# ushasigh/srsran-edgeric-5g

Measured on AMD Instinct MI355X. Metric: pdsch_slots_per_sec, higher is better.
Workload: dtype u32 bit-packed GF(2) + bf16 grid + f32 IQ

## Files before the change

### srsran-edgeric-5g_amd/csrc/ldpc_device.h

```cpp
#pragma once

#include "bits_device.h"

namespace nrphy {

constexpr int LDPC_MAX_WPB   = 12;
constexpr int LDPC_LIN_WORDS = (68 * 384) / 32 + 2;
constexpr int LDPC_DBL_WORDS = 2 * 22 * LDPC_MAX_WPB;

template <bool ALIGNED>
__device__ __forceinline__ uint32_t rot_word(const uint32_t* a, uint32_t base, uint32_t zc, uint32_t s, uint32_t j)
{
  uint32_t start = s + 32u * j;
  start          = start >= zc ? start - zc : start;
  if (ALIGNED) {
    const uint32_t wpb = zc >> 5, bw = base >> 5;
    const uint32_t w0 = start >> 5, sh = s & 31u;
    const uint32_t w1 = (w0 + 1u == wpb) ? 0u : w0 + 1u;
    return (a[bw + w0] << sh) | ((a[bw + w1] >> 1) >> (31u - sh));
  }
  uint32_t n_valid = zc - 32u * j;
  n_valid          = n_valid > 32u ? 32u : n_valid;
  uint32_t first   = zc - start;
  first            = first > n_valid ? n_valid : first;
  uint32_t v       = ext32(a, base + start) & topmask(first);
  if (first < n_valid) {
    v |= (ext32(a, base) & topmask(n_valid - first)) >> first;
  }
  return v;
}

struct LdpcScratch {
  uint32_t aux[4][LDPC_MAX_WPB + 1];
  uint32_t sum[LDPC_MAX_WPB + 2];
  uint32_t p0[LDPC_MAX_WPB + 2];
};

template <bool ALIGNED>
__device__ __forceinline__ void put_block_word(uint32_t* lin, uint32_t node, uint32_t zc, uint32_t j, uint32_t v)
{
  uint32_t pos = node * zc + 32u * j;
  if (ALIGNED) {
    lin[pos >> 5] = v;
  } else {
    uint32_t n_valid = zc - 32u * j;
    or_bits_lds(lin, pos, v, n_valid > 32u ? 32u : n_valid);
  }
}

constexpr uint32_t LDPC_GRAPH_ROWPTR = 48;

__device__ __forceinline__ void stage_graph(const LiftedGraph* g, uint32_t nof_rows, uint32_t* gbuf, uint32_t lane)
{
  if (lane <= nof_rows) {
    gbuf[lane] = g->row_ptr[lane];
  }
  const uint32_t nedges = g->row_ptr[nof_rows];
  for (uint32_t e = lane; e < nedges; e += WAVE) {
    gbuf[LDPC_GRAPH_ROWPTR + e] = g->edge[e];
  }
}

struct GraphRows {
  static constexpr uint32_t TRIPS = (MAX_BG_EDGES + WAVE - 1) / WAVE;
  uint32_t row_ptr, nedges, edge[TRIPS];
  __device__ __forceinline__ void fetch(const LiftedGraph* g, uint32_t nof_rows, uint32_t lane)
  {
    row_ptr = lane <= nof_rows ? g->row_ptr[lane] : 0u;
    nedges  = g->row_ptr[nof_rows];
#pragma unroll
    for (uint32_t k = 0; k != TRIPS; ++k) {
      edge[k] = lane + WAVE * k < nedges ? g->edge[lane + WAVE * k] : 0u;
    }
  }
  __device__ __forceinline__ void store(uint32_t nof_rows, uint32_t* gbuf, uint32_t lane) const
  {
    if (lane <= nof_rows) {
      gbuf[lane] = row_ptr;
    }
#pragma unroll
    for (uint32_t k = 0; k != TRIPS; ++k) {
      if (lane + WAVE * k < nedges) {
        gbuf[LDPC_GRAPH_ROWPTR + lane + WAVE * k] = edge[k];
      }
    }
  }
};

template <bool ALIGNED>
__device__ __forceinline__ uint32_t row_word(const uint32_t* gbuf, const uint32_t* lin, uint32_t zc, uint32_t m,
                                             uint32_t j)
{
  uint32_t acc = 0;
  for (uint32_t e = gbuf[m], end = gbuf[m + 1]; e != end; ++e) {
    uint32_t edge = gbuf[LDPC_GRAPH_ROWPTR + e];
    acc ^= rot_word<ALIGNED>(lin, edge >> 16, zc, edge & 0xFFFFu, j);
  }
  return acc;
}

__device__ __forceinline__ uint32_t core_row_word_dbl(const uint32_t* gbuf, const uint32_t* dbl, uint32_t m, uint32_t j)
{
  uint32_t       acc = 0;
  const uint8_t* at  = reinterpret_cast<const uint8_t*>(dbl) + 4u * j;
  uint32_t       e = gbuf[m], end = gbuf[m + 1];
  for (; e + 4u <= end; e += 4u) {
    uint32_t        edge[4];
    u32x2_unaligned w[4];
#pragma unroll
    for (int k = 0; k != 4; ++k) {
      edge[k] = gbuf[LDPC_GRAPH_ROWPTR + e + k];
    }
#pragma unroll
    for (int k = 0; k != 4; ++k) {
      w[k] = *reinterpret_cast<const u32x2_unaligned*>(at + (edge[k] >> 16));
    }
#pragma unroll
    for (int k = 0; k != 4; ++k) {
      acc ^= __builtin_amdgcn_alignbit(w[k].x, w[k].y, edge[k]);
    }
  }
  for (; e != end; ++e) {
    const uint32_t        edge = gbuf[LDPC_GRAPH_ROWPTR + e];
    const u32x2_unaligned w    = *reinterpret_cast<const u32x2_unaligned*>(at + (edge >> 16));
    acc ^= __builtin_amdgcn_alignbit(w.x, w.y, edge);
  }
  return acc;
}

__device__ __forceinline__ void ldpc_double_blocks(const uint32_t* lin, uint32_t kb, uint32_t wpb, uint32_t* dbl, uint32_t lane)
{
  const uint32_t magic = (65536u + wpb - 1u) / wpb;
  for (uint32_t item = lane; item < kb * wpb; item += WAVE) {
    const uint32_t n = __umul24(item, magic) >> 16;
    const uint32_t v = lin[item];
    dbl[item + __umul24(n, wpb)]       = v;
    dbl[item + __umul24(n, wpb) + wpb] = v;
  }
}

template <bool ALIGNED>
__device__ inline void ldpc_encode_wave_impl(const LiftedGraph* g, const uint32_t* gbuf, uint32_t kb, uint32_t zc,
                                             uint32_t nof_rows, uint32_t* lin, uint32_t* dbl, LdpcScratch* sc, uint32_t lane)
{
  const uint32_t wpb = (zc + 31u) >> 5;
  if (ALIGNED) {
    ldpc_double_blocks(lin, kb, wpb, dbl, lane);
    wave_sync();
  }
  const uint32_t wpb_magic = (65536u + wpb - 1u) / wpb;
  for (uint32_t item = lane; item < 4u * wpb; item += WAVE) {
    const uint32_t m = __umul24(item, wpb_magic) >> 16, j = item - __umul24(m, wpb);
    sc->aux[m][j] = ALIGNED ? core_row_word_dbl(gbuf, dbl, m, j) : row_word<ALIGNED>(gbuf, lin, zc, m, j);
  }
  wave_sync();
  if (lane < wpb) {
    sc->sum[lane] = sc->aux[0][lane] ^ sc->aux[1][lane] ^ sc->aux[2][lane] ^ sc->aux[3][lane];
  }
  if (lane == 0) {
    sc->sum[wpb] = 0;
    sc->p0[wpb]  = 0;
  }
  wave_sync();
  uint32_t p0w = 0;
  if (lane < wpb) {
    uint32_t b = g->core_b;
    p0w        = rot_word<ALIGNED>(sc->sum, 0, zc, b == 0 ? 0 : zc - b, lane);
    sc->p0[lane] = p0w;
  }
  wave_sync();
  if (lane < wpb) {
    uint32_t p1 = sc->aux[0][lane] ^ rot_word<ALIGNED>(sc->p0, 0, zc, g->core_s0, lane);
    uint32_t p3 = sc->aux[3][lane] ^ rot_word<ALIGNED>(sc->p0, 0, zc, g->core_s3, lane);
    uint32_t p2 = (g->core_mid == 1) ? (sc->aux[2][lane] ^ p3) : (sc->aux[1][lane] ^ p1);
    put_block_word<ALIGNED>(lin, kb + 0, zc, lane, p0w);
    put_block_word<ALIGNED>(lin, kb + 1, zc, lane, p1);
    put_block_word<ALIGNED>(lin, kb + 2, zc, lane, p2);
    put_block_word<ALIGNED>(lin, kb + 3, zc, lane, p3);
  }
  wave_sync();
  uint32_t ext_items = (nof_rows > 4u ? nof_rows - 4u : 0u) * wpb;
  for (uint32_t item = lane; item < ext_items; item += WAVE) {
    uint32_t m = item / wpb, j = item - m * wpb;
    m += 4u;
    put_block_word<ALIGNED>(lin, kb + m, zc, j, row_word<ALIGNED>(gbuf, lin, zc, m, j));
  }
  wave_sync();
}

__device__ inline void ldpc_encode_wave(const LiftedGraph* g, const uint32_t* gbuf, uint32_t kb, uint32_t zc,
                                        uint32_t nof_rows, uint32_t* lin, uint32_t* dbl, LdpcScratch* sc, uint32_t lane)
{
  if ((zc & 31u) == 0) {
    ldpc_encode_wave_impl<true>(g, gbuf, kb, zc, nof_rows, lin, dbl, sc, lane);
  } else {
    ldpc_encode_wave_impl<false>(g, gbuf, kb, zc, nof_rows, lin, dbl, sc, lane);
  }
}

}
```

### srsran-edgeric-5g_amd/csrc/nrphy_host.cpp

```cpp
#include "nrphy_host_internal.h"
#include "nrphy_trace.h"

#include <algorithm>
#include <cmath>
#include <complex>
#include <cstdlib>
#include <cstring>
#include <array>
#include <map>
#include <mutex>
#include <new>
#include <unordered_map>
#include <vector>

using namespace nrphy;

namespace {

struct nr_ldpc_edge_t {
  uint8_t  row;
  uint8_t  col;
  uint16_t shift[8];
};
#include "nr_ldpc_bg.inc"
// ... 682 lines not shown
}

extern "C" int nrphy_destroy(nrphy_ctx_t* ctx)
{
  if (ctx == nullptr) {
    return NRPHY_OK;
  }
  (void)hipSetDevice(ctx->device);
  (void)hipFree(ctx->d_graphs);
  (void)hipFree(ctx->d_gold);
  (void)hipFree(ctx->d_tbcrc);
  for (void* b : ctx->scratch) {
    (void)hipFree(b);
  }
  for (DecoderGraph* g : ctx->d_dec_graph) {
    (void)hipFree(g);
  }
  for (uint32_t* a : ctx->d_dec_addr) {
    (void)hipFree(a);
  }
  for (auto& kv : ctx->d_dec_crc) {
    (void)hipFree(kv.second);
  }
  for (auto& kv : ctx->d_tb_crc_w) {
    (void)hipFree(kv.second);
  }
  (void)hipFree(ctx->d_x1);
  (void)hipFree(ctx->d_prach);
  for (auto& kv : ctx->d_twiddle) {
    (void)hipFree(kv.second);
  }
  if (ctx->stream) {
    (void)hipStreamDestroy(ctx->stream);
  }
  delete ctx;
  return NRPHY_OK;
}

extern "C" int nrphy_synchronize(nrphy_ctx_t* ctx, void* stream)
{
  if (ctx == nullptr) {
    return NRPHY_ERR_ARGUMENT;
  }
  HIP_TRY(hipStreamSynchronize(stream ? (hipStream_t)stream : ctx->stream));
  return NRPHY_OK;
}

const float2* get_twiddle(nrphy_ctx* ctx, uint32_t size)
{
  if (!dft_size_supported(size)) {
    return nullptr;
  }
  std::lock_guard<std::recursive_mutex> lock(ctx->host_mutex);
  auto it = ctx->d_twiddle.find(size);
  if (it != ctx->d_twiddle.end()) {
    return it->second;
  }
  std::vector<float2> tw(size);
  for (uint32_t k = 0; k != size; ++k) {
    double ang = 2.0 * M_PI * (double)k / (double)size;
    tw[k]      = make_float2((float)std::cos(ang), (float)std::sin(ang));
  }
  float2* d = nullptr;
  if (upload(&d, tw.data(), tw.size() * sizeof(float2)) != hipSuccess) {
    return nullptr;
  }
  ctx->d_twiddle[size] = d;
  return d;
}

namespace {

void append_allocation_signature(const nrphy_pdsch_pdu_t& pdu, std::vector<uint64_t>& sig)
{
  sig.insert(sig.end(), std::begin(pdu.prb_mask), std::end(pdu.prb_mask));
  sig.push_back(((uint64_t)pdu.start_symbol_index << 48) | ((uint64_t)pdu.nof_symbols << 40) |
                ((uint64_t)pdu.nof_cdm_groups_without_data << 36) | ((uint64_t)pdu.nof_layers << 32) |
                pdu.dmrs_symbol_mask);
  sig.push_back(((uint64_t)pdu.bwp_start_rb << 32) | ((uint64_t)pdu.bwp_size_rb << 8) | pdu.nof_reserved);
  for (unsigned r = 0; r != pdu.nof_reserved; ++r) {
    sig.insert(sig.end(), std::begin(pdu.reserved[r].prb_mask), std::end(pdu.reserved[r].prb_mask));
    sig.push_back(((uint64_t)pdu.reserved[r].re_mask << 32) | pdu.reserved[r].symbol_mask);
  }
}

struct ReMapping {
  uint32_t sym_re_start[NRPHY_NSYMB + 1];
  uint32_t sym_kind[NRPHY_NSYMB];
  uint32_t sym_arg[NRPHY_NSYMB];
};

}

struct PlanShapeCache {
  struct Remap {
    ReMapping             m;
    std::vector<uint16_t> table;
  };
  struct Zero {
    std::vector<ZeroSeg> segs;
    uint32_t             nof_long = 0;
  };
  std::map<std::vector<uint64_t>, Remap> remap;
  std::map<std::vector<uint64_t>, Zero>  zero;
  static constexpr size_t MAX_ENTRIES = 256;
};

PlanShapeCache* plan_shape_cache_create()
{
  return new (std::nothrow) PlanShapeCache;
}
void plan_shape_cache_destroy(PlanShapeCache* c)
{
  delete c;
}

namespace {

struct EncodeOnly {
  uint32_t nof_re;
  uint32_t nref;
};

int plan_create(nrphy_ctx_t* ctx, uint32_t n_pdu, const nrphy_pdsch_pdu_t* pdus, const uint64_t* tb_offset,
                const uint32_t* grid_index, uint32_t nof_grids, uint32_t grid_nof_ports, uint32_t grid_nof_subc,
                const EncodeOnly* enc, nrphy_pdsch_plan_t** out, PlanPlacement* place = nullptr);

}

int nrphy_pdsch_plan_create_placed(nrphy_ctx_t* ctx, uint32_t n_pdu, const nrphy_pdsch_pdu_t* pdus, const uint64_t* tb_offset,
                                   const uint32_t* grid_index, uint32_t nof_grids, uint32_t grid_nof_ports,
                                   uint32_t grid_nof_subc, PlanPlacement* place, nrphy_pdsch_plan_t** out)
{
  return plan_create(ctx, n_pdu, pdus, tb_offset, grid_index, nof_grids, grid_nof_ports, grid_nof_subc, nullptr, out, place);
}

extern "C" int nrphy_pdsch_plan_create(nrphy_ctx_t* ctx, uint32_t n_pdu, const nrphy_pdsch_pdu_t* pdus,
                                       const uint64_t* tb_offset, const uint32_t* grid_index, uint32_t nof_grids,
                                       uint32_t grid_nof_ports, uint32_t grid_nof_subc, nrphy_pdsch_plan_t** out)
{
  return plan_create(ctx, n_pdu, pdus, tb_offset, grid_index, nof_grids, grid_nof_ports, grid_nof_subc, nullptr, out);
}

namespace {

int plan_create(nrphy_ctx_t* ctx, uint32_t n_pdu, const nrphy_pdsch_pdu_t* pdus, const uint64_t* tb_offset,
                const uint32_t* grid_index, uint32_t nof_grids, uint32_t grid_nof_ports, uint32_t grid_nof_subc,
                const EncodeOnly* enc, nrphy_pdsch_plan_t** out, PlanPlacement* place)
{
  if (ctx == nullptr || out == nullptr || (n_pdu != 0 && (pdus == nullptr || tb_offset == nullptr)) ||
      grid_nof_ports == 0 || grid_nof_ports > NRPHY_MAX_PORTS || grid_nof_subc == 0 || grid_nof_subc % 12 != 0 ||
      grid_nof_subc > NRPHY_MAX_RB * 12) {
    return NRPHY_ERR_ARGUMENT;
  }
  *out = nullptr;
  if (place == nullptr) {
    HIP_TRY(hipSetDevice(ctx->device));
  }
  nrphy_pdsch_plan* plan = new (std::nothrow) nrphy_pdsch_plan;
  if (plan == nullptr) {
    return NRPHY_ERR_CAPACITY;
  }
  PlanShapeCache* shapes = place ? place->cache : nullptr;
  if (shapes != nullptr && shapes->remap.size() + shapes->zero.size() > PlanShapeCache::MAX_ENTRIES) {
    shapes->remap.clear();
    shapes->zero.clear();
  }
  plan->ctx            = ctx;
  plan->nof_grids      = nof_grids;
  plan->grid_nof_ports = grid_nof_ports;
  plan->grid_nof_subc  = grid_nof_subc;
  plan->encode_only    = enc != nullptr;

  std::vector<CbWork>   work;
  std::vector<DmrsWork> dmrs;
  std::vector<CrcWork>  crc_work;
  std::vector<uint64_t> remap_sig;
  std::map<std::vector<uint64_t>, ReMapping> remap_cache;
  std::vector<ScrWork>  scr_work;
  std::unordered_map<SeqKey, SeqShare, SeqKeyHash> seq_shares;
  std::vector<uint8_t>  seq_fresh;
  uint32_t              seed_slots = 0;
  uint64_t              seq_words = 0;
  uint64_t              seq_words_sum = 0;
  bool                  seq_words_fit = true;
  std::vector<std::vector<uint32_t>> pdus_of_grid(nof_grids);
  std::vector<float>    weights;
  std::vector<uint16_t> re_table;
  std::vector<uint8_t>  mask(grid_nof_subc);
  std::vector<uint16_t> list;
  uint64_t              cw_bits = 0;
  int                   status  = NRPHY_OK;

  for (uint32_t i = 0; i != n_pdu && status == NRPHY_OK; ++i) {
    const nrphy_pdsch_pdu_t& pdu = pdus[i];
    if (enc == nullptr ? nrphy_pdsch_validate(&pdu) != NRPHY_OK
                       : (pdu.qm < 2 || pdu.qm > 8 || (pdu.qm & 1U) || pdu.rv > 3 || pdu.nof_layers == 0 ||
                          pdu.nof_layers > NRPHY_MAX_LAYERS || pdu.tb_size_bytes == 0 ||
                          pdu.tb_size_bytes > NRPHY_MAX_TB_BYTES || (pdu.ldpc_base_graph != 1 && pdu.ldpc_base_graph != 2))) {
      status = NRPHY_ERR_INVALID_PDU;
      break;
    }
    const uint32_t g = grid_index ? grid_index[i] : 0;
    if (g >= nof_grids || pdu.nof_ports > grid_nof_ports || (tb_offset[i] & 3U) != 0 ||
        (enc == nullptr && 12U * (unsigned)(mask_highest(pdu.prb_mask) + 1) > grid_nof_subc)) {
      status = NRPHY_ERR_ARGUMENT;
      break;
    }
    PduDev pd;
    std::memset(&pd, 0, sizeof(pd));
    unsigned nof_re = 0;
    remap_sig.clear();
    append_allocation_signature(pdu, remap_sig);
    auto cached = remap_cache.find(remap_sig);
    if (enc != nullptr) {
      nof_re = enc[i].nof_re;
      for (unsigned l = 0; l <= NRPHY_NSYMB; ++l) {
        pd.sym_re_start[l] = (l == NRPHY_NSYMB) ? nof_re : 0;
      }
    } else if (cached != remap_cache.end()) {
      std::memcpy(pd.sym_re_start, cached->second.sym_re_start, sizeof(pd.sym_re_start));
      std::memcpy(pd.sym_kind, cached->second.sym_kind, sizeof(pd.sym_kind));
      std::memcpy(pd.sym_arg, cached->second.sym_arg, sizeof(pd.sym_arg));
      nof_re = pd.sym_re_start[NRPHY_NSYMB];
    } else {
      PlanShapeCache::Remap        built;
      const PlanShapeCache::Remap* rel = nullptr;
      if (shapes != nullptr) {
        auto known = shapes->remap.find(remap_sig);
        if (known != shapes->remap.end()) {
          rel = &known->second;
        }
      }
      if (rel == nullptr) {
        for (unsigned l = 0; l != NRPHY_NSYMB; ++l) {
          built.m.sym_re_start[l] = nof_re;
          built.m.sym_arg[l]      = 0;
          data_re_mask(pdu, l, mask);
          list.clear();
          for (unsigned k = 0; k != grid_nof_subc; ++k) {
            if (mask[k]) {
              list.push_back((uint16_t)k);
            }
          }
          if (list.empty()) {
            built.m.sym_kind[l] = SYM_NONE;
          } else if ((unsigned)(list.back() - list.front()) + 1 == list.size()) {
            built.m.sym_kind[l] = SYM_CONTIGUOUS;
            built.m.sym_arg[l]  = list.front();
          } else {
            built.m.sym_kind[l] = SYM_TABLE;
            built.m.sym_arg[l]  = (uint32_t)built.table.size();
            for (unsigned lp = 0; lp != l; ++lp) {
              if (built.m.sym_kind[lp] == SYM_TABLE && built.m.sym_re_start[lp + 1] - built.m.sym_re_start[lp] == list.size() &&
                  std::equal(list.begin(), list.end(), built.table.begin() + built.m.sym_arg[lp])) {
                built.m.sym_arg[l] = built.m.sym_arg[lp];
                break;
              }
            }
            if (built.m.sym_arg[l] == built.table.size()) {
              built.table.insert(built.table.end(), list.begin(), list.end());
            }
          }
          nof_re += (unsigned)list.size();
          built.m.sym_re_start[l + 1] = nof_re;
        }
        rel = &built;
        if (shapes != nullptr) {
          rel = &shapes->remap.insert({remap_sig, built}).first->second;
        }
      }
      const uint32_t base = (uint32_t)re_table.size();
      re_table.insert(re_table.end(), rel->table.begin(), rel->table.end());
      std::memcpy(pd.sym_re_start, rel->m.sym_re_start, sizeof(pd.sym_re_start));
      std::memcpy(pd.sym_kind, rel->m.sym_kind, sizeof(pd.sym_kind));
      for (unsigned l = 0; l != NRPHY_NSYMB; ++l) {
        pd.sym_arg[l] = rel->m.sym_arg[l] + (rel->m.sym_kind[l] == SYM_TABLE ? base : 0U);
      }
      nof_re = pd.sym_re_start[NRPHY_NSYMB];
      ReMapping m;
      std::memcpy(m.sym_re_start, pd.sym_re_start, sizeof(m.sym_re_start));
      std::memcpy(m.sym_kind, pd.sym_kind, sizeof(m.sym_kind));
      std::memcpy(m.sym_arg, pd.sym_arg, sizeof(m.sym_arg));
      remap_cache.insert({remap_sig, m});
    }
    if (nof_re == 0) {
      status = NRPHY_ERR_INVALID_PDU;
      break;
    }
    nrphy_pdsch_derived_t d;
    derive(pdu, nof_re, d, enc ? &enc[i].nref : nullptr);
    if (d.lifting_size == 0 || d.nof_codeblocks > NRPHY_MAX_CODEBLOCKS || d.nof_codeblocks > nof_re ||
        d.rm_length_short == 0) {
      status = NRPHY_ERR_INVALID_PDU;
      break;
    }
    const unsigned kb = (pdu.ldpc_base_graph == 1) ? 22 : 10;
    pd.tb_offset      = tb_offset[i];
    pd.cw_bit_offset  = cw_bits;
    pd.tb_bytes       = pdu.tb_size_bytes;
    pd.grid_index     = g;
    pd.graph          = (pdu.ldpc_base_graph - 1) * NOF_LIFTING_SIZES + (uint32_t)lifting_position(d.lifting_size);
    pd.zc             = d.lifting_size;
    pd.kb             = kb;
    pd.K              = d.segment_length;
    pd.info_bits      = d.cb_info_bits;
    pd.filler         = d.nof_filler_bits;
    pd.tb_crc_bits    = d.nof_tb_crc_bits;
    pd.cb_crc_bits    = d.nof_cb_crc_bits;
    pd.zero_pad       = d.zero_pad;
    pd.C              = d.nof_codeblocks;
    pd.n_short        = d.nof_short_segments;
    pd.e_short        = d.rm_length_short;
    pd.e_long         = d.rm_length_long;
    pd.n_cb           = d.n_cb;
    pd.k0             = d.k0;
    pd.qm             = pdu.qm;
    pd.nof_layers     = pdu.nof_layers;
    pd.nof_ports      = pdu.nof_ports;
    pd.c_init         = (pdu.rnti << 15) + pdu.n_id;
    pd.nof_re         = nof_re;
    {
      const unsigned nsys = (kb - 2) * d.lifting_size;
      unsigned       fs = std::min(nsys - d.nof_filler_bits, d.n_cb), fe = std::min(nsys, d.n_cb);
      const unsigned flen = fe - fs, n_valid = d.n_cb - flen;
      const unsigned rank0 = d.k0 < fs ? d.k0 : (d.k0 < fe ? fs : d.k0 - flen);
      unsigned       last;
      if (rank0 + d.rm_length_long > n_valid) {
        last = d.n_cb - 1;
      } else {
        unsigned u = rank0 + d.rm_length_long - 1;
        last       = u < fs ? u : u + flen;
      }
      const unsigned nodes = divide_ceil(last + 1 + 2 * d.lifting_size, d.lifting_size);
      pd.nof_rows          = std::max(4U, nodes > kb ? nodes - kb : 0U);
    }
    {
      const float avg     = (pdu.qm == 2) ? 2.0F : (pdu.qm == 4) ? 10.0F : (pdu.qm == 6) ? 42.0F : 170.0F;
      float       scaling = std::sqrt(1 / avg);
      const float cfg     = std::pow(10.0F, -pdu.ratio_pdsch_data_to_sss_dB / 20.0F);
      if (std::isnormal(cfg)) {
        scaling *= cfg;
      }
      const unsigned nw      = 2 * pdu.nof_prg * pdu.nof_ports * pdu.nof_layers;
      pd.weights_offset      = (uint32_t)weights.size();
      for (unsigned k = 0; k != nw; ++k) {
        weights.push_back(pdu.precoding ? pdu.precoding[k] * scaling : 0.0F);
      }
      pd.dmrs_weights_offset = (uint32_t)weights.size();
      for (unsigned k = 0; k != nw; ++k) {
        weights.push_back(pdu.precoding ? pdu.precoding[k] : 0.0F);
      }
      pd.nof_prg       = pdu.nof_prg;
      pd.prg_size_subc = pdu.prg_size_rb * 12;
    }
    pd.dmrs_symbol_mask = pdu.dmrs_symbol_mask;
    pd.dmrs_zero_other_group = (pdu.nof_cdm_groups_without_data == 2 && (pdu.nof_layers + 1) / 2 == 1) ? 1U : 0U;
    pd.dmrs_ref_rb      = (pdu.ref_point == 1) ? pdu.bwp_start_rb : 0;
    {
      const float amp   = std::pow(10.0F, -pdu.ratio_pdsch_dmrs_to_sss_dB / 20.0F);
      pd.dmrs_amplitude = (float)(M_SQRT1_2 * (double)amp);
    }
    for (unsigned l = 0; l != NRPHY_NSYMB; ++l) {
      const uint64_t a  = (uint64_t)(14 * pdu.slot_index + l + 1) * (2 * pdu.scrambling_id + 1);
      pd.dmrs_c_init[l] = (uint32_t)(((a << 17) + (2 * pdu.scrambling_id + (pdu.n_scid ? 1 : 0))) & 0x7FFFFFFFULL);
      if ((pdu.dmrs_symbol_mask >> l) & 1U) {
        const uint32_t first = (uint32_t)mask_lowest(pdu.prb_mask), end = (uint32_t)mask_highest(pdu.prb_mask) + 1;
        for (uint32_t b = first; b < end; b += DMRS_PRB_CHUNK) {
          dmrs.push_back({i, l, b, std::min<uint32_t>(end, b + DMRS_PRB_CHUNK)});
        }
      }
    }
    for (unsigned w = 0; w != NRPHY_PRB_WORDS; ++w) {
      pd.prb_mask[2 * w]     = (uint32_t)pdu.prb_mask[w];
      pd.prb_mask[2 * w + 1] = (uint32_t)(pdu.prb_mask[w] >> 32);
    }
    pd.first_prb = (uint32_t)mask_lowest(pdu.prb_mask);
    pd.end_prb   = (uint32_t)mask_highest(pdu.prb_mask) + 1;
    if (pdu.nof_cdm_groups_without_data < (pdu.nof_layers + 1) / 2) {
      plan->dmrs_separate = true;
    }
    pdus_of_grid[g].push_back(i);
    const unsigned lq = pdu.nof_layers * pdu.qm;
    const size_t   work_before = work.size();
    for (unsigned cb = 0; cb != d.nof_codeblocks; ++cb) {
      const unsigned nre = ((cb < d.nof_short_segments) ? d.rm_length_short : d.rm_length_long) / lq;
      for (unsigned begin = 0; begin < nre; begin += RE_CHUNK) {
        const unsigned count = std::min<unsigned>(RE_CHUNK, nre - begin);
        work.push_back({i, cb, begin, count});
        {
          const uint64_t bit0 = (uint64_t)(cb < d.nof_short_segments ? cb * d.rm_length_short
                                                                     : d.nof_short_segments * d.rm_length_short +
                                                                           (cb - d.nof_short_segments) * d.rm_length_long) +
                                (uint64_t)begin * lq;
          const uint32_t need = std::max<uint32_t>(31U, (uint32_t)(((bit0 & 31U) + (uint64_t)count * lq + 31U) / 32U) + 1U);
          plan->lds_lin_words = std::max<uint32_t>(plan->lds_lin_words, (need + 3U) & ~3U);
        }
        plan->lds_symb_words = std::max<uint32_t>(plan->lds_symb_words,
                                                  (((count * pdu.nof_layers + 31) / 32) * 8 + 8 + 3) & ~3U);
      }
    }
    plan->lds_lin_words = std::max<uint32_t>(plan->lds_lin_words,
                                             ((((kb + pd.nof_rows) * d.lifting_size + 31) / 32) + 2 + 3) & ~3U);
    plan->lds_graph_words = std::max<uint32_t>(
        plan->lds_graph_words, (48U + ctx->graphs[pd.graph].row_ptr[std::min<uint32_t>(pd.nof_rows, MAX_BG_ROWS)] + 3U) & ~3U);
    pd.scr_words  = (d.codeword_bits + 31U) / 32U + 1U + 31U;
    pd.dmrs_seq_words  = (12U * (pd.end_prb - pd.dmrs_ref_rb) + 31U) / 32U + 1U;
    {
      const uint32_t nof_dmrs_words = (uint32_t)(((uint64_t)pd.dmrs_seq_words * (unsigned)__builtin_popcount(pdu.dmrs_symbol_mask) + 3U) & ~3ULL);
      const uint32_t nof_items      = (uint32_t)(work.size() - work_before);
      uint8_t        fresh          = (uint8_t)(SEQ_NEW_SCR | (nof_dmrs_words != 0 ? SEQ_NEW_DMRS : 0));
      SeqShare       share          = {seed_slots, (uint32_t)seq_words, (uint32_t)plan->scr_words};
      if (n_pdu != 1) {
        SeqKey key;
        key.scr  = {pd.c_init, pd.C, pd.n_short, pd.e_short, pd.e_long, lq};
        key.dmrs = {};
        key.dmrs[0] = pdu.dmrs_symbol_mask;
        key.dmrs[1] = pd.dmrs_seq_words;
        for (unsigned l = 0; l != NRPHY_NSYMB; ++l) {
          key.dmrs[2 + l] = ((pdu.dmrs_symbol_mask >> l) & 1U) ? pd.dmrs_c_init[l] : 0U;
        }
        auto both = seq_shares.find(key);
        if (both != seq_shares.end()) {
          share = both->second;
          fresh = 0;
        } else {
          SeqKey half = key;
          half.dmrs   = {};
          half.dmrs[1] = ~0U;
          auto scr_known = seq_shares.insert({half, share});
          if (!scr_known.second) {
            share.seed_first      = scr_known.first->second.seed_first;
            share.scr_word_offset = scr_known.first->second.scr_word_offset;
            fresh &= (uint8_t)~SEQ_NEW_SCR;
          }
          if (nof_dmrs_words != 0) {
            half     = key;
            half.scr = {};
            auto dmrs_known = seq_shares.insert({half, share});
            if (!dmrs_known.second) {
              share.dmrs_seq_offset = dmrs_known.first->second.dmrs_seq_offset;
              fresh &= (uint8_t)~SEQ_NEW_DMRS;
            }
          }
          seq_shares.insert({key, share});
        }
      }
      pd.seed_first      = share.seed_first;
      pd.scr_word_offset = share.scr_word_offset;
      pd.dmrs_seq_offset = share.dmrs_seq_offset;
      if (fresh & SEQ_NEW_SCR) {
        seed_slots += nof_items;
        seq_words_sum += pd.scr_words;
        seq_words += (pd.scr_words + 15U) & ~15ULL;
        seq_words_fit = seq_words_fit && pd.scr_words <= (uint32_t)GOLD_X1_WORDS && seq_words <= 0xFFFFFFFFULL;
        ++plan->n_scr_seq;
      }
      if (fresh & SEQ_NEW_DMRS) {
        plan->scr_words += nof_dmrs_words;
        ++plan->n_dmrs_seq;
      }
      seq_fresh.push_back(fresh);
    }
    plan->n_cb += d.nof_codeblocks;
    plan->cw_offset.push_back(cw_bits);
    cw_bits += (d.codeword_bits + 31U) & ~31ULL;
    plan->pdus.push_back(pd);
  }
  if (status == NRPHY_OK) {
    const uint32_t parts_big = ctx->tune.scr_parts_big > 0 ? (uint32_t)std::min((int)SCR_PARTS, ctx->tune.scr_parts_big) : 1U;
    const uint32_t parts_max = plan->n_scr_seq >= 128 ? parts_big : SCR_PARTS;
    for (uint32_t i = 0; i != n_pdu; ++i) {
      const PduDev&  pd       = plan->pdus[i];
      const uint32_t own_dmrs = (seq_fresh[i] & SEQ_NEW_DMRS) ? 1U : 0U;
      if (seq_fresh[i] & SEQ_NEW_SCR) {
        const uint32_t parts = std::min<uint32_t>(parts_max, std::max<uint32_t>(1, pd.scr_words >> 11));
        const uint32_t chunk = divide_ceil(pd.scr_words, parts);
        for (uint32_t first = 0, k = 0; first < pd.scr_words; first += chunk, ++k) {
          scr_work.push_back({i, first, std::min(chunk, pd.scr_words - first), k == 0 ? own_dmrs : 0U});
        }
      } else if (own_dmrs) {
        scr_work.push_back({i, 0U, 0U, 1U});
      }
    }
  }
  for (uint32_t i = 0; i != n_pdu && status == NRPHY_OK; ++i) {
    PduDev&         pd = plan->pdus[i];
    const CrcField& f  = (pd.tb_crc_bits == 16) ? CRC16_FIELD : CRC24A_FIELD;
    const uint32_t  n  = pd.tb_bytes;
    const uint32_t  regions = divide_ceil(n, TB_CRC_REGION_BYTES);
    const uint32_t  want  = std::max<uint32_t>(1, std::min<uint32_t>(regions, TB_CRC_TARGET_WORK / std::max<uint32_t>(1, n_pdu)));
    uint32_t        per   = std::min<uint32_t>(TB_CRC_MAX_REGIONS_PER_WORK, divide_ceil(regions, want));
    if (ctx->tune.crc_regions > 0) {
      per = std::max(1, std::min((int)TB_CRC_MAX_REGIONS_PER_WORK, ctx->tune.crc_regions));
    }
    pd.crc_first      = (uint32_t)crc_work.size();
    pd.crc_count      = divide_ceil(regions, per);
    if (pd.crc_count > 64) {
      status = NRPHY_ERR_INVALID_PDU;
      break;
    }
    for (uint32_t region = 0; region < regions; region += per) {
      const uint32_t count      = std::min(per, regions - region);
      const int64_t  region_end = (int64_t)(region + count) * TB_CRC_REGION_BYTES;
      crc_work.push_back({i, region, f.xpow((int64_t)f.order + 8 * ((int64_t)n - region_end)), count});
    }
  }
  if (status != NRPHY_OK) {
    delete plan;
    return status;
  }
  std::vector<ZeroWork> zero_work;
  std::vector<ZeroSeg>  zero_segs;
  {
    std::map<std::vector<uint64_t>, std::array<uint32_t, 3>> seen;
    std::vector<uint8_t>  cov((size_t)NRPHY_NSYMB * grid_nof_subc);
    std::vector<uint64_t> key, sig;
    std::map<std::vector<uint64_t>, std::array<uint32_t, 3>> by_signature;
    for (uint32_t g = 0; g != (enc ? 0U : nof_grids); ++g) {
      for (uint32_t port = 0; port != grid_nof_ports; ++port) {
        sig.clear();
        for (uint32_t i : pdus_of_grid[g]) {
          const nrphy_pdsch_pdu_t& pdu = pdus[i];
          if (port >= pdu.nof_ports) {
            continue;
          }
          append_allocation_signature(pdu, sig);
        }
        auto known = by_signature.find(sig);
        if (known != by_signature.end()) {
          if (known->second[1] != 0) {
            zero_work.push_back({g, port, known->second[0], known->second[1], known->second[2]});
          }
          continue;
        }
        if (shapes != nullptr) {
          sig.push_back(((uint64_t)grid_nof_subc << 32) | port);
          auto kept = shapes->zero.find(sig);
          sig.pop_back();
          if (kept != shapes->zero.end()) {
            const std::array<uint32_t, 3> where = {(uint32_t)zero_segs.size(), (uint32_t)kept->second.segs.size(),
                                                   kept->second.nof_long};
            zero_segs.insert(zero_segs.end(), kept->second.segs.begin(), kept->second.segs.end());
            by_signature.insert({sig, where});
            if (where[1] != 0) {
              zero_work.push_back({g, port, where[0], where[1], where[2]});
            }
            continue;
          }
        }
        std::fill(cov.begin(), cov.end(), 0);
        for (uint32_t i : pdus_of_grid[g]) {
          const nrphy_pdsch_pdu_t& pdu = pdus[i];
          if (port >= pdu.nof_ports) {
            continue;
          }
          for (unsigned l = 0; l != NRPHY_NSYMB; ++l) {
            uint8_t* row = &cov[(size_t)l * grid_nof_subc];
            data_re_mask(pdu, l, mask);
            for (unsigned k = 0; k != grid_nof_subc; ++k) {
              row[k] |= mask[k];
            }
            if ((pdu.dmrs_symbol_mask >> l) & 1U) {
              const unsigned groups = (pdu.nof_cdm_groups_without_data == 2) ? 2 : (pdu.nof_layers + 1) / 2;
              for (unsigned prb = 0; 12 * prb < grid_nof_subc; ++prb) {
                if (mask_test(pdu.prb_mask, prb)) {
                  for (unsigned k = 0; k != 12; ++k) {
                    row[12 * prb + k] |= (k % 2) < groups;
                  }
                }
              }
            }
          }
        }
        key.clear();
        for (unsigned l = 0; l != NRPHY_NSYMB; ++l) {
          const uint8_t* row = &cov[(size_t)l * grid_nof_subc];
          unsigned       k   = 0;
          while (k < grid_nof_subc) {
            if (row[k]) {
              ++k;
              continue;
            }
            unsigned k0 = k;
            while (k < grid_nof_subc && !row[k]) {
              ++k;
            }
            key.push_back(((uint64_t)l << 32) | ((uint64_t)k0 << 16) | (k - k0));
          }
        }
        if (key.empty()) {
          by_signature.insert({sig, {0, 0, 0}});
          if (shapes != nullptr) {
            sig.push_back(((uint64_t)grid_nof_subc << 32) | port);
            shapes->zero.insert({sig, PlanShapeCache::Zero()});
            sig.pop_back();
          }
          continue;
        }
        auto it = seen.find(key);
        if (it == seen.end()) {
          const uint32_t begin = (uint32_t)zero_segs.size();
          uint32_t       nof_long = 0;
          for (int pass = 0; pass != 2; ++pass) {
            for (uint64_t v : key) {
              const bool is_long = (v & 0xFFFF) >= ZERO_LONG_RUN;
// ... 2323 lines not shown
```

### srsran-edgeric-5g_amd/csrc/nrphy_internal.h

```cpp
#pragma once

#include "mi355_nrphy.h"

#include <hip/hip_runtime.h>
#include <stdint.h>

namespace nrphy {

constexpr int NOF_LIFTING_SIZES = 51;
constexpr int NOF_GRAPHS        = 2 * NOF_LIFTING_SIZES;
constexpr int MAX_BG_ROWS       = 46;
constexpr int MAX_BG_EDGES      = 316;

struct LiftedGraph {
  uint16_t row_ptr[MAX_BG_ROWS + 2];
  uint16_t core_b;
  uint16_t core_s0;
  uint16_t core_s3;
  uint16_t core_mid;
  uint32_t edge[MAX_BG_EDGES];
};

#define NR_POLAR_SUBBLOCK_PATTERN                                                                                       \
  {0, 1, 2, 4, 3, 5, 6, 7, 8, 16, 9, 17, 10, 18, 11, 19, 12, 20, 13, 21, 14, 22, 15, 23, 24, 25, 26, 28, 27, 29, 30, 31}

constexpr int GOLD_JUMP_BITS  = 24;
constexpr int GOLD_X1_WORDS   = 1 << 16;

constexpr uint32_t SCR_PARTS = 4;

constexpr int CRC_POW_WORDS = 288;

struct GoldTables {
  uint32_t x2_jump[GOLD_JUMP_BITS][32];
  uint32_t x2_head[32][32];
  uint32_t crc24b_pow32[CRC_POW_WORDS];
  uint32_t crc24b_table[256];
  uint32_t crc24b_slice[4][256];
  uint32_t crc24b_mul[CRC_POW_WORDS][6][16];
  float2 qam_lut[4][256];
};

constexpr int RE_CHUNK = 512;
#ifndef NRPHY_CRC_SLICES
#define NRPHY_CRC_SLICES 3
#endif
#define NRPHY_CB_U_GRAPH_OFFSET (2 * 22 * 12 + 80)

enum SymKind : uint32_t { SYM_NONE = 0, SYM_CONTIGUOUS = 1, SYM_TABLE = 2 };

struct PduDev {
  uint64_t tb_offset;
  uint64_t cw_bit_offset;
  uint32_t tb_bytes;
  uint32_t grid_index;
  uint32_t graph;
  uint32_t zc;
  uint32_t kb;
  uint32_t K;
  uint32_t info_bits;
  uint32_t filler;
  uint32_t tb_crc_bits;
  uint32_t cb_crc_bits;
  uint32_t zero_pad;
  uint32_t C;
  uint32_t n_short;
  uint32_t e_short;
  uint32_t e_long;
  uint32_t n_cb;
  uint32_t k0;
  uint32_t nof_rows;
  uint32_t qm;
  uint32_t nof_layers;
  uint32_t nof_ports;
  uint32_t c_init;
  uint32_t item_first;
  uint32_t seed_first;
  uint32_t scr_words;
  uint32_t scr_word_offset;
  uint32_t nof_re;
  uint32_t weights_offset;
  uint32_t dmrs_weights_offset;
  uint32_t nof_prg;
  uint32_t prg_size_subc;
  uint32_t sym_re_start[NRPHY_NSYMB + 1];
  uint32_t sym_kind[NRPHY_NSYMB];
  uint32_t sym_arg[NRPHY_NSYMB];
  uint32_t dmrs_symbol_mask;
  uint32_t dmrs_zero_other_group;
  uint32_t dmrs_c_init[NRPHY_NSYMB];
  uint32_t dmrs_ref_rb;
  uint32_t dmrs_seq_offset;
  uint32_t dmrs_seq_words;
  float    dmrs_amplitude;
  uint32_t prb_mask[2 * NRPHY_PRB_WORDS];
  uint32_t first_prb;
  uint32_t end_prb;
  uint32_t crc_first;
  uint32_t crc_count;
};

struct CbWork {
  uint32_t pdu;
  uint32_t cb;
  uint32_t re_begin;
  uint32_t re_count;
};

constexpr int DMRS_PRB_CHUNK = 32;
#ifndef NRPHY_CRC_WORDS_PER_THREAD
#define NRPHY_CRC_WORDS_PER_THREAD 16
#endif
constexpr uint32_t TB_CRC_REGION_WORDS = 256 * NRPHY_CRC_WORDS_PER_THREAD;
constexpr uint32_t TB_CRC_REGION_BYTES = 4 * TB_CRC_REGION_WORDS;

struct TbCrcTables {
  uint32_t y32[2][4][256];
  uint32_t y1k[2][4][256];
  uint32_t y8k[2][4][256];
  uint32_t yz[2][4][256];
  uint32_t lane[2][64];
};

struct DmrsWork {
  uint32_t pdu;
  uint32_t symbol;
  uint32_t prb_begin;
  uint32_t prb_end;
};

struct ScrWork {
  uint32_t pdu;
  uint32_t first;
  uint32_t count;
  uint32_t with_dmrs;
};

struct CrcWork {
  uint32_t pdu;
  uint32_t region;
  uint32_t factor;
  uint32_t count;
};
constexpr uint32_t TB_CRC_MAX_REGIONS_PER_WORK = 8;
constexpr uint32_t TB_CRC_TARGET_WORK          = 1024;

struct ZeroSeg {
  uint16_t symbol;
  uint16_t k0;
  uint16_t count;
  uint16_t pad_;
};
constexpr uint32_t ZERO_LONG_RUN = 32;
struct ZeroWork {
  uint32_t grid;
  uint32_t port;
  uint32_t seg_begin;
  uint32_t seg_count;
  uint32_t seg_long;
};

struct PdschLaunch {
  const ZeroWork*    zero_work;
  const ZeroSeg*     zero_segs;
  uint32_t           n_zero_work;
  uint32_t           n_dmrs_in_launch;
  uint32_t*          scr;
  uint32_t*          scr_seq;
  uint32_t           scr_as_words;
  const PduDev*      pdus;
  const CbWork*      work;
  const DmrsWork*    dmrs_work;
  const CrcWork*     crc_work;
  const ScrWork*     scr_work;
  uint32_t           n_scr_work;
  const TbCrcTables* tbcrc;
  uint32_t           n_crc_work;
  const float*       weights;
  const uint16_t*    re_table;
  const LiftedGraph* graphs;
  const GoldTables*  gold;
  const uint32_t*    x1_words;
  uint32_t*          tb_crc_part;
  uint32_t           n_pdu;
  uint32_t           n_work;
  uint32_t           work_base;
  uint32_t           n_dmrs_work;
  uint32_t           grid_nof_ports;
  uint32_t           grid_nof_subc;
  uint32_t           lds_lin_words;
  uint32_t           lds_u_words;
  uint32_t           profile_stage;
  uint32_t           extras_nt;
  uint32_t           prologue_order;
  uint32_t           zero_fill;
};

hipError_t launch_prologue(const PdschLaunch& p, const uint8_t* d_tb, hipStream_t stream);
constexpr uint32_t CB_BUCKETS        = 16;
constexpr uint32_t CB_MIXED_MAX_WORK = 4096;
inline uint32_t cb_bucket(uint32_t qm, uint32_t nof_layers)
{
  return (qm / 2u - 1u) * 4u + (nof_layers - 1u);
}
bool       codeblocks_take_bucket_launches(const PdschLaunch& p, const uint32_t* bucket_begin, int dispatch, uint32_t* nof_buckets);
hipError_t launch_codeblocks(const PdschLaunch& p, const uint32_t* bucket_begin, int dispatch, const uint8_t* d_tb,
                             uint32_t* d_grid, uint32_t* d_cw_rm, uint32_t* d_cw_scr, const hipStream_t* streams, uint32_t n_streams);
hipError_t launch_dmrs(const PdschLaunch& p, uint32_t* d_grid, hipStream_t stream);
hipError_t launch_ldpc_encode(const LiftedGraph* graphs, uint32_t graph, uint32_t kb, uint32_t zc, uint32_t n_cb,
                              const uint8_t* d_msg, uint32_t msg_stride, uint32_t out_bits, uint8_t* d_out,
                              uint32_t out_stride, hipStream_t stream);

struct DecoderGraph {
  uint32_t row_ptr[MAX_BG_ROWS + 2];
  uint32_t pair_ptr[MAX_BG_ROWS + 2];
  uint32_t quad_ptr[MAX_BG_ROWS + 2];
  uint32_t edge[MAX_BG_EDGES];
};

constexpr uint32_t DEC_CRC_TABLE_WORDS = 8 * 16;

struct LdpcDecodeLaunch {
  const DecoderGraph* graph;
  const uint32_t*     pair_addr;
  const int8_t*       llr;
  uint2*              scratch;
  uint32_t*           slot_flags;
  uint32_t            nof_slots;
  uint32_t            slot_bytes;
  uint8_t*            out;
  uint32_t*           iterations;
  const uint32_t*     crc_weight;
  const uint8_t*      skip;
  uint8_t*            ok_flags;
  uint32_t            crc_at_end;
  uint32_t            zc, bg_k, nof_nodes, nof_layers_max;
  uint32_t            nof_llr, llr_stride, out_stride, nof_filler;
  uint32_t            crc_poly, crc_order;
  uint32_t            max_iterations;
  float               scaling_factor;
  uint32_t            lm_lds_bytes;
  uint32_t            lds_tail_off;
  uint32_t            scale_arithmetic;
  uint32_t            scale_fixed;
  int                 knob_pairs, knob_ldsmsg;
};
hipError_t launch_ldpc_decode(const LdpcDecodeLaunch& p, uint32_t n_cb, hipStream_t stream);

enum DematchKind : uint32_t { DEMATCH_ZERO = 0, DEMATCH_FILL, DEMATCH_COPY, DEMATCH_COMBINE };
struct DematchOp {
  uint32_t kind, begin, count, src;
};
constexpr uint32_t MAX_DEMATCH_OPS = 60;
struct DematchLaunch {
  const int8_t* in;
  int8_t*       out;
  uint32_t      in_stride, out_stride, block_length, qm, cols, n_ops;
  uint32_t      in_stride_outer, out_stride_outer;
  uint32_t      skip_load;
  uint32_t      disjoint;
  const DematchOp* ops_ext;
  DematchOp        ops[MAX_DEMATCH_OPS];
};
hipError_t launch_ldpc_dematch(const DematchLaunch& p, uint32_t n_cb, hipStream_t stream, uint32_t n_outer = 1);

struct PuschAssembleLaunch {
  const uint8_t* cb_msg;
  uint8_t*       cb_ok;
  const uint32_t* cb_iter;
  const uint8_t* skipped;
  uint8_t*       tb;
  uint32_t*      result;
  const uint32_t* crc_weight;
  const TbCrcTables* tbcrc;
  uint32_t       crc_factor;
  uint32_t       C, msg_stride, tb_stride, tb_bytes, cb_info_bits, max_iterations;
};
constexpr uint32_t PUSCH_ASSEMBLE_THREADS = 1024;
hipError_t launch_pusch_assemble(const PuschAssembleLaunch& p, uint32_t n_tb, hipStream_t stream);

constexpr uint32_t CSI_RS_MAX_SEQ_WORDS = 128;
struct CsiRsWork {
  uint32_t grid_index, symbol, c_init;
  uint32_t advance, seq_len;
  uint32_t rb_begin, rb_stride, re_mask, n_re_prb;
  uint32_t nof_ports, first_layer, group_size;
  uint32_t weights_offset;
  float    amplitude;
};
struct CsiRsLaunch {
  const CsiRsWork*  work;
  const float*      weights;
  const GoldTables* gold;
  const uint32_t*   x1_words;
  uint32_t*         grid;
  uint32_t          grid_nof_ports, grid_nof_subc;
};
hipError_t launch_csi_rs(const CsiRsLaunch& p, uint32_t n_work, hipStream_t stream);
hipError_t launch_llr_descramble(const GoldTables* gold, const uint32_t* x1_words, const uint32_t* d_c_init, uint32_t n_cw,
                                 uint32_t length, const int8_t* d_in, size_t in_stride, int8_t* d_out, size_t out_stride,
                                 hipStream_t stream);
constexpr uint32_t DEMOD_MAX_PAIRS = 4;
struct DemodLaunch {
  uint32_t modulation;
  uint32_t span_len;
  uint32_t nof_vector;
  float    range, scale;
  float    qam16_gain, qam16_threshold;
  uint32_t nof_intervals[DEMOD_MAX_PAIRS];
  float    width[DEMOD_MAX_PAIRS], rcp_width[DEMOD_MAX_PAIRS];
  float    slope[DEMOD_MAX_PAIRS][16], intercept[DEMOD_MAX_PAIRS][16];
};
hipError_t launch_demodulate_soft(const DemodLaunch& p, uint32_t nof_spans, const float* d_symbols, const float* d_noise,
                                  int8_t* d_llr, hipStream_t stream);
bool demod_params(uint32_t modulation, uint32_t span_len, DemodLaunch& p);

constexpr uint32_t PUSCH_DEMOD_THREADS = 256;
struct PuschDemodDesc {
  uint32_t grid_index, nof_rx_ports, nof_layers, qm;
  uint32_t equalizer, c_init, prb_first, dmrs_re_per_prb;
  uint32_t rx_ports[NRPHY_MAX_PORTS];
  uint8_t  dmrs_subc[NRPHY_NRE];
  uint32_t item_first, nof_items;
  uint64_t ce_offset;
};
struct PuschDemodItem {
  uint32_t pusch, symbol, dmrs;
  uint32_t re_first, count;
  uint32_t bit_offset;
  uint32_t span_pos, nof_vector;
};
struct PuschDemodLaunch {
  const PuschDemodDesc* desc;
  const PuschDemodItem* items;
  const uint16_t*       prbs;
  const DemodLaunch*    demod;
  const GoldTables*     gold;
  const uint32_t*       x1_words;
  const uint32_t*       grid;
  const uint32_t*       ch;
  const float*          noise;
  int8_t*               llr;
  uint64_t              llr_stride;
  double*               partial;
  float*                sinr;
  uint32_t              grid_nof_ports, grid_nof_subc, n_pusch, n_items;
};
hipError_t launch_pusch_demod(const PuschDemodLaunch& p, hipStream_t stream);
struct EqualizeLaunch {
  uint32_t        algorithm, n_batch, nof_re, nof_layers, nof_rx_ports;
  float           tx_scaling;
  const uint32_t* rx;
  const uint32_t* ch;
  const float*    noise;
  float*          eq;
  float*          eq_nvars;
};
hipError_t launch_channel_equalize(const EqualizeLaunch& p, hipStream_t stream);
constexpr uint32_t PUSCH_CHEST_TA_WINDOW  = 144;
constexpr uint32_t PUSCH_CHEST_MAX_LAYERS = 2;
struct PuschChestDesc {
  uint32_t grid_index, nof_rx_ports, nof_layers, nprb;
  uint32_t prb_first;
  uint32_t first_symbol, nof_symbols, nof_dmrs;
  uint32_t nwords;
  uint32_t ntaps, nof_v;
  uint32_t dc;
  uint32_t scs_hz;
  uint32_t rx_ports[NRPHY_MAX_PORTS];
  uint32_t dmrs_symbol[NRPHY_NSYMB];
  uint32_t c_init[NRPHY_NSYMB];
  float    epoch[NRPHY_NSYMB];
  float    taps[16];
  float    beta, ls_scale;
  uint64_t ce_offset;
  uint64_t row_offset;
};
struct PuschChestLaunch {
  const PuschChestDesc*     desc;
  const uint32_t*           jobs;
  const uint16_t*           prbs;
  const float2*             twiddle;
  const GoldTables*         gold;
  const uint32_t*           x1_words;
  const uint32_t*           grid;
  uint32_t*                 ch;
  float*                    noise_vars;
  nrphy_pusch_chest_meas_t* meas;
  uint32_t*                 rows;
  float2*                   rot;
  uint32_t                  grid_nof_ports, grid_nof_subc, n_jobs;
};
hipError_t launch_pusch_chest(const PuschChestLaunch& p, hipStream_t stream);
constexpr uint32_t PRACH_L_LONG = 839, PRACH_L_SHORT = 139, PRACH_N_LONG = 1024, PRACH_N_SHORT = 256;
struct PrachTables {
  float2 cexp_long[4 * PRACH_L_LONG];
  float2 cexp_short[4 * PRACH_L_SHORT];
  float2 tw_long[PRACH_N_LONG];
  float2 tw_short[PRACH_N_SHORT];
};
struct PrachSequence {
  uint16_t u, factor, offset, shift;
// ... 326 lines not shown
```

### srsran-edgeric-5g_amd/csrc/pdsch_kernels.hip

```cpp
#include "ldpc_device.h"

#ifndef NRPHY_PHASE_A_STAGED
#define NRPHY_PHASE_A_STAGED 1
#endif

#ifdef NRPHY_PROBES
#define NRPHY_STAGE(p) ((p).profile_stage)
#else
#define NRPHY_STAGE(p) 0u
#endif

namespace nrphy {

__global__ __launch_bounds__(TB_CRC_THREADS) void prologue_kernel(PdschLaunch p, const uint8_t* __restrict__ d_tb)
{
  constexpr uint32_t LDS_WORDS = TB_CRC_LDS_WORDS;
  __shared__ __attribute__((aligned(16))) uint32_t lds[LDS_WORDS];
  static_assert(LDS_WORDS >= GOLD_RING_WORDS, "LDS of the sequence role");
  const uint32_t tid = threadIdx.x;

  uint32_t scr_index = blockIdx.x, crc_index = blockIdx.x - p.n_scr_work;
  bool     scr_role  = blockIdx.x < p.n_scr_work;
  if (p.prologue_order == 1 && p.n_scr_work != 0 && p.n_crc_work != 0) {
    const uint32_t total = p.n_scr_work + p.n_crc_work;
    const uint32_t xcd = blockIdx.x & 7u, turn = blockIdx.x >> 3, q = total >> 3, r = total & 7u;
    const uint32_t pos = xcd * q + (xcd < r ? xcd : r) + turn;
    const uint32_t s0 = (uint32_t)(((uint64_t)pos * p.n_scr_work + total - 1u) / total);
    const uint32_t s1 = (uint32_t)(((uint64_t)(pos + 1u) * p.n_scr_work + total - 1u) / total);
    scr_role  = s1 > s0;
    scr_index = s0;
    crc_index = pos - s0;
  }
  NRPHY_WG_TRACE_MARK(0);
  NRPHY_WG_TRACE_WHERE(scr_role ? 1 : 2);
  if (scr_role) {
    if (NRPHY_STAGE(p) == 8) {
      return;
    }
    const auto*    swc   = to_constant(&p.scr_work[scr_index]);
    const uint32_t first = swc->first, count = swc->count;
    const bool     with_dmrs = swc->with_dmrs != 0;
    PduRef         pd    = *to_constant(&p.pdus[swc->pdu]);
    const uint32_t wave = tid / WAVE, lane = tid % WAVE;
    constexpr uint32_t DMRS_WAVES = TB_CRC_THREADS / WAVE - 1, DMRS_SCRATCH = (GOLD_RING_WORDS - 2048u) / DMRS_WAVES;
    static_assert(GOLD_SEED_WORDS <= 2048u && GOLD_RING_WORDS > 2048u, "LDS of the sequence role");
    static_assert((12u * NRPHY_MAX_RB + 31u) / 32u + 1u <= DMRS_SCRATCH, "DM-RS scratch per wave");
    if (wave == 0) {
      if (count == 0) {
        return;
      }
      if (p.scr_as_words != 0) {
        constexpr uint32_t SCR_STORE_ROWS = 8;
        uint32_t*       out = p.scr_seq + pd.scr_word_offset + first;
        const uint32_t* x1  = p.x1_words + first;
        gold_sequence_blocks_wave(p.gold, pd.c_init, first, count, lds, lane, [&](uint32_t base, uint32_t avail) {
          for (uint32_t k0 = lane; k0 < avail; k0 += SCR_STORE_ROWS * WAVE) {
            uint32_t x[SCR_STORE_ROWS];
#pragma unroll
            for (uint32_t i = 0; i != SCR_STORE_ROWS; ++i) {
              const uint32_t k = k0 + i * WAVE;
              x[i]             = k < avail ? x1[base + k] : 0u;
            }
#pragma unroll
            for (uint32_t i = 0; i != SCR_STORE_ROWS; ++i) {
              const uint32_t k = k0 + i * WAVE;
              if (k < avail) {
                out[base + k] = lds[k] ^ x[i];
              }
            }
          }
        });
        NRPHY_WG_TRACE_MARK(6);
        return;
      }
      const uint32_t lq = pd.qm * pd.nof_layers, n_short = pd.n_short, e_short = pd.e_short, e_long = pd.e_long, C = pd.C;
      const uint32_t nre_short = e_short / lq, nre_long = e_long / lq;
      struct Cursor {
        uint32_t cb, re_begin, item, bit_cb, nre;
      };
      Cursor resume = {0u, 0u, pd.seed_first, 0u, n_short != 0 ? nre_short : nre_long};
      auto   advance = [&](Cursor& c) {
        c.re_begin += RE_CHUNK;
        if (c.re_begin >= c.nre) {
          c.bit_cb += c.cb < n_short ? e_short : e_long;
          ++c.cb;
          c.re_begin = 0;
          c.nre      = c.cb < n_short ? nre_short : nre_long;
        }
        ++c.item;
      };
      gold_sequence_blocks_wave(p.gold, pd.c_init, first, count, lds, lane, [&](uint32_t base, uint32_t avail) {
        const uint32_t lo = first + base, hi = lo + avail;
        Cursor c        = resume;
        bool   resuming = false;
        while (c.cb < C) {
          const uint32_t w0 = (c.bit_cb + c.re_begin * lq) >> 5;
          if (w0 >= hi) {
            break;
          }
          if (w0 + 31u > lo) {
            const uint32_t k = w0 + lane;
            if (lane < 31u && k >= lo && k < hi) {
              p.scr_seq[(size_t)c.item * 32u + lane] = lds[k - lo];
            }
          }
          if (w0 + 31u > hi && !resuming) {
            resume   = c;
            resuming = true;
          }
          advance(c);
        }
        if (!resuming) {
          resume = c;
        }
      });
      NRPHY_WG_TRACE_MARK(6);
    } else if (with_dmrs && pd.dmrs_seq_words <= DMRS_SCRATCH) {
      uint32_t ordinal = 0;
      for (uint32_t mask = pd.dmrs_symbol_mask; mask != 0; mask &= mask - 1u, ++ordinal) {
        if (ordinal % DMRS_WAVES == wave - 1u) {
          const uint32_t l = (uint32_t)__ffs(mask) - 1u;
          gold_sequence_wave(p.gold, p.x1_words, pd.dmrs_c_init[l], pd.dmrs_seq_words,
                             p.scr + pd.dmrs_seq_offset + ordinal * pd.dmrs_seq_words,
                             lds + 2048u + (wave - 1u) * DMRS_SCRATCH, lane);
        }
      }
    }
    return;
  }

  if (NRPHY_STAGE(p) == 9) {
    return;
  }
  const auto*     wkc = to_constant(&p.crc_work[crc_index]);
  const uint32_t  wk_pdu = wkc->pdu, wk_region = wkc->region, wk_factor = wkc->factor, wk_count = wkc->count;
  PduRef          pd  = *to_constant(&p.pdus[wk_pdu]);
  const uint32_t  sel = (pd.tb_crc_bits == 16) ? 1u : 0u;
  const CrcPoly   c   = sel ? crc16() : crc24a();
  const uint32_t  n   = pd.tb_bytes;
  const uint32_t* tbw = reinterpret_cast<const uint32_t*>(d_tb + pd.tb_offset);
#ifdef NRPHY_WG_TRACE
  asm volatile("s_waitcnt lgkmcnt(0)" ::: "memory");
  NRPHY_WG_TRACE_MARK(3);
#endif
  const uint32_t share = tbcrc_regions_workgroup(p.tbcrc, sel, c, tbw, n, wk_region, wk_count, wk_factor, lds, tid);
  if (tid == 0) {
    p.tb_crc_part[crc_index] = share;
  }
  NRPHY_WG_TRACE_MARK(6);
}

#ifdef NRPHY_WG_TRACE
extern "C" int nrphy_debug_wg_trace(uint64_t* out, uint32_t nof_blocks)
{
  const size_t n = 8 * (size_t)(nof_blocks < WG_TRACE_MAX ? nof_blocks : WG_TRACE_MAX) * sizeof(uint64_t);
  return (int)hipMemcpyFromSymbol(out, HIP_SYMBOL(g_wg_trace), n, 0, hipMemcpyDeviceToHost);
}
#endif

hipError_t launch_prologue(const PdschLaunch& p, const uint8_t* d_tb, hipStream_t stream)
{
  if (p.n_crc_work + p.n_scr_work == 0) {
    return hipSuccess;
  }
  hipLaunchKernelGGL(prologue_kernel, dim3(p.n_crc_work + p.n_scr_work), dim3(TB_CRC_THREADS), 0, stream, p, d_tb);
  return hipGetLastError();
}

constexpr uint32_t CB_U_QAM_WORDS     = 512;
constexpr uint32_t CB_U_LDPC_WORDS    = (sizeof(LdpcScratch) / 4u + 3u) & ~3u;
constexpr uint32_t CB_U_GRAPH_OFFSET  = LDPC_DBL_WORDS + CB_U_LDPC_WORDS;
static_assert(CB_U_GRAPH_OFFSET == NRPHY_CB_U_GRAPH_OFFSET, "host and device agree on the layout of the scratch region");

struct CbShared {
  uint32_t* lin;
  uint32_t* u;
  uint32_t* symb;
  uint32_t* graph;
  LdpcScratch* ldpc;
};

#ifndef NRPHY_LDS_PROBE
#define NRPHY_LDS_PROBE 0
#endif
__device__ __forceinline__ uint32_t lds_probe_index(uint32_t idx, uint32_t bit)
{
  if ((NRPHY_LDS_PROBE >> bit) & 1) {
    uint32_t zero = 0;
    asm volatile("" : "+v"(zero));
    const uint32_t lane = __builtin_amdgcn_mbcnt_hi(~0u, __builtin_amdgcn_mbcnt_lo(~0u, 0u));
    return (idx & zero) + lane;
  }
  return idx;
}

__device__ __forceinline__ uint32_t crc24_word_step(const uint32_t* tab, uint32_t reg, uint32_t word)
{
#if NRPHY_CRC_SLICES == 4
  const uint32_t v = (reg << 8) ^ word;
  return tab[v & 0xFFu] ^ tab[256u + ((v >> 8) & 0xFFu)] ^ tab[512u + ((v >> 16) & 0xFFu)] ^ tab[768u + (v >> 24)];
#else
  const uint32_t v = reg ^ (word >> 8);
  uint32_t       r = tab[lds_probe_index(v & 0xFFu, 1)] ^ tab[256u + lds_probe_index((v >> 8) & 0xFFu, 1)] ^ tab[512u + lds_probe_index(v >> 16, 1)];
  return ((r << 8) & 0xFFFFFFu) ^ tab[lds_probe_index(((r >> 16) ^ word) & 0xFFu, 1)];
#endif
}

__device__ inline void build_codeblock(PduRef pd, uint32_t cb, const uint32_t* tbw, const uint32_t* tb_crc_part,
                                       const GoldTables* tables, CbShared* sh, uint32_t total_words, uint32_t lane,
                                       uint32_t profile_stage)
{
  const bool     last    = (cb == pd.C - 1);
  const uint32_t used    = pd.info_bits - (last ? pd.tb_crc_bits + pd.zero_pad : 0u);
  const uint32_t tb_pos  = cb * pd.info_bits;
  const uint32_t tb_bits = pd.tb_bytes * 8u;
  const uint4* crc_src = reinterpret_cast<const uint4*>(&tables->crc24b_slice[0][0]);
  const uint4  crc_tab0 = crc_src[lane], crc_tab1 = crc_src[lane + WAVE], crc_tab2 = crc_src[lane + 2 * WAVE];
#if NRPHY_CRC_SLICES == 4
  const uint4 crc_tab3 = crc_src[lane + 3 * WAVE];
#endif
  constexpr uint32_t SEG_UNROLL = 5;
  for (uint32_t base = lane; base < total_words; base += WAVE * SEG_UNROLL) {
    uint32_t hi[SEG_UNROLL], lo[SEG_UNROLL];
#pragma unroll
    for (uint32_t k = 0; k != SEG_UNROLL; ++k) {
      const uint32_t pos = 32u * (base + WAVE * k);
      hi[k] = 0;
      lo[k] = 0;
      if (pos < used) {
        const uint32_t abs_pos = tb_pos + pos;
        const uint32_t i = abs_pos >> 5, sft = abs_pos & 31u;
        hi[k] = tbw[i];
        if (sft != 0 && 32u * (i + 1) < tb_bits) {
          lo[k] = tbw[i + 1];
        }
      }
    }
#pragma unroll
    for (uint32_t k = 0; k != SEG_UNROLL; ++k) {
      const uint32_t j = base + WAVE * k, pos = 32u * j;
      if (j < total_words) {
        uint32_t v = 0;
        if (pos < used) {
          v = __funnelshift_l(__builtin_bswap32(lo[k]), __builtin_bswap32(hi[k]), (tb_pos + pos) & 31u);
          const uint32_t remaining = used - pos;
          if (remaining < 32u) {
            v &= topmask(remaining);
          }
        }
        sh->lin[j] = v;
      }
    }
  }
  {
    uint4* dst           = reinterpret_cast<uint4*>(sh->u);
    dst[lane]            = crc_tab0;
    dst[lane + WAVE]     = crc_tab1;
    dst[lane + 2 * WAVE] = crc_tab2;
#if NRPHY_CRC_SLICES == 4
    dst[lane + 3 * WAVE] = crc_tab3;
#endif
  }
  wave_sync();
  if (profile_stage == 7) {
    return;
  }
  if (last) {
    const uint32_t tb_crc = wave_xor(lane < pd.crc_count ? tb_crc_part[pd.crc_first + lane] : 0u);
    if (lane == 0) {
      or_bits_lds_exclusive(sh->lin, used, tb_crc << (32u - pd.tb_crc_bits), pd.tb_crc_bits);
    }
  }
  wave_sync();
  if (pd.cb_crc_bits) {
    const uint32_t n   = pd.info_bits;
    const uint32_t pad = (32u - (n & 31u)) & 31u;
    const uint32_t nw  = (n + pad) >> 5;
    const uint32_t per = (nw + WAVE - 1) / WAVE;
    uint32_t       a   = lane * per;
    uint32_t       b   = a + per;
    a                  = a > nw ? nw : a;
    b                  = b > nw ? nw : b;
    uint32_t reg       = 0;
    for (uint32_t j = a; j < b; ++j) {
      uint32_t word;
      if (pad == 0) {
        word = sh->lin[j];
      } else if (j == 0) {
        word = sh->lin[0] >> pad;
      } else {
        word = ext32(sh->lin, 32u * j - pad);
      }
      reg = crc24_word_step(sh->u, reg, word);
    }
    uint32_t part = 0;
    {
      const uint32_t m = nw - b;
#pragma unroll
      for (uint32_t k = 0; k != 6; ++k) {
        part ^= tables->crc24b_mul[m][k][(reg >> (4u * k)) & 15u];
      }
    }
    uint32_t crc = wave_xor(part);
    if (lane == 0) {
      or_bits_lds_exclusive(sh->lin, n, crc << 8, 24);
    }
    wave_sync();
  }
}

struct RmIndex {
  uint32_t fs;
  uint32_t flen;
  uint32_t n_valid;
  uint32_t rank0;
  float    inv_valid;
};

__device__ __forceinline__ RmIndex rm_index_init(PduRef pd)
{
  RmIndex  r;
  uint32_t nsys = (pd.kb - 2u) * pd.zc;
  uint32_t fs   = nsys - pd.filler;
  uint32_t fe   = nsys;
  fs            = fs > pd.n_cb ? pd.n_cb : fs;
  fe            = fe > pd.n_cb ? pd.n_cb : fe;
  r.fs          = fs;
  r.flen        = fe - fs;
  r.n_valid     = pd.n_cb - r.flen;
  r.rank0       = pd.k0 < fs ? pd.k0 : (pd.k0 < fe ? fs : pd.k0 - r.flen);
  r.inv_valid   = 1.0f / (float)r.n_valid;
  return r;
}

template <bool WRAP>
__device__ __forceinline__ uint32_t rm_gather32(const RmIndex& r, const uint32_t* lin, uint32_t zc2, uint32_t t)
{
  uint32_t u = r.rank0 + t;
  if (WRAP && u >= r.n_valid) {
    uint32_t q = (uint32_t)((float)u * r.inv_valid);
    u -= q * r.n_valid;
    if ((int32_t)u < 0) {
      u += r.n_valid;
    } else if (u >= r.n_valid) {
      u -= r.n_valid;
    }
  }
  uint32_t run = (u < r.fs) ? r.fs - u : r.n_valid - u;
  uint32_t out = ext32(lin, (u < r.fs ? u : u + r.flen) + zc2);
  if (run >= 32u) {
    return out;
  }
  out &= topmask(run);
  uint32_t filled = run;
  while (filled < 32u) {
    u += run;
    if (u >= r.n_valid) {
      if (!WRAP) {
        break;
      }
      u = 0;
    }
    run            = (u < r.fs) ? r.fs - u : r.n_valid - u;
    run            = run > 32u - filled ? 32u - filled : run;
    uint32_t piece = ext32(lin, (u < r.fs ? u : u + r.flen) + zc2);
    out |= (piece & topmask(run)) >> filled;
    filled += run;
  }
  return out;
}

__device__ __forceinline__ uint32_t bit_select(uint32_t m, uint32_t a, uint32_t b)
{
  return __builtin_amdgcn_bitop3_b32(m, a, b, 0xCA);
}

__device__ __forceinline__ void transpose8x8(uint32_t& hi, uint32_t& lo)
{
  hi = bit_select(0xAA55AA55u, hi, bit_select(0x55005500u, hi << 7, hi >> 7));
  lo = bit_select(0xAA55AA55u, lo, bit_select(0x55005500u, lo << 7, lo >> 7));
  hi = bit_select(0xCCCC3333u, hi, bit_select(0x33330000u, hi << 14, hi >> 14));
  lo = bit_select(0xCCCC3333u, lo, bit_select(0x33330000u, lo << 14, lo >> 14));
  const uint32_t nhi = bit_select(0xF0F0F0F0u, hi, lo >> 4);
  const uint32_t nlo = bit_select(0x0F0F0F0Fu, lo, hi << 4);
  hi                 = nhi;
  lo                 = nlo;
}

__device__ __forceinline__ void cmul_ref(float xr, float xi, float wr, float wi, float& outr, float& outi)
{
  float t0 = __fmul_rn(xi, wi);
  float t1 = __fmul_rn(xr, wi);
  outr     = __fmaf_rn(xr, wr, -t0);
  outi     = __fmaf_rn(xi, wr, t1);
}

typedef float cf2 __attribute__((ext_vector_type(2)));
__device__ __forceinline__ cf2 cmul_ref_packed(cf2 x, cf2 w)
{
  cf2 t, r;
  asm("v_pk_mul_f32 %0, %1, %2 op_sel:[1,1] op_sel_hi:[0,1]" : "=v"(t) : "v"(x), "v"(w));
  asm("v_pk_fma_f32 %0, %1, %2, %3 op_sel_hi:[1,0,1] neg_lo:[0,0,1]" : "=v"(r) : "v"(x), "v"(w), "v"(t));
  return r;
}
__device__ __forceinline__ cf2 cmul_ref_packed_uniform(cf2 x, cf2 w)
{
  cf2 t, r;
  asm("v_pk_mul_f32 %0, %1, %2 op_sel:[1,1] op_sel_hi:[0,1]" : "=v"(t) : "v"(x), "s"(w));
  asm("v_pk_fma_f32 %0, %1, %2, %3 op_sel_hi:[1,0,1] neg_lo:[0,0,1]" : "=v"(r) : "v"(x), "s"(w), "v"(t));
  return r;
}

typedef __bf16 bf16x2_t __attribute__((ext_vector_type(2)));
typedef float  f32x2_t __attribute__((ext_vector_type(2)));
__device__ __forceinline__ uint32_t pack_cbf16(float re, float im)
{
  f32x2_t  v = {re, im};
  bf16x2_t b = __builtin_convertvector(v, bf16x2_t);
  return *reinterpret_cast<uint32_t*>(&b);
}

__device__ __forceinline__ void grid_store(uint32_t* p, uint32_t v)
{
  __builtin_nontemporal_store(v, p);
}

#ifndef NRPHY_GRID_STORE_AUX
#define NRPHY_GRID_STORE_AUX 2
#endif
#ifndef NRPHY_GRID_BUFFER_STORES
#define NRPHY_GRID_BUFFER_STORES 1
#endif

struct ChunkGeom {
  uint32_t E;
  uint32_t cw_cb;
  uint32_t bit0;
};

template <int QM, int L, bool WRAP>
__device__ __forceinline__ void phase_a(const PdschLaunch& p, PduRef pd, const CbWork& wk, const CbShared& sh,
                                        uint32_t E, uint32_t lane)
{
  const uint32_t esym = E / QM;
  const uint32_t zc2  = 2u * pd.zc;
  const RmIndex  rm   = rm_index_init(pd);
  const uint32_t s0   = wk.re_begin * L;
  const uint32_t nblk = (wk.re_count * L + 31u) >> 5;
  constexpr uint32_t LUT_TRIPS = ((1u << QM) + WAVE - 1u) / WAVE;
  float2             lut[LUT_TRIPS];
#pragma unroll
  for (uint32_t k = 0; k != LUT_TRIPS; ++k) {
    lut[k] = lane + WAVE * k < (1u << QM) ? p.gold->qam_lut[QM / 2 - 1][lane + WAVE * k] : make_float2(0.f, 0.f);
  }
#if NRPHY_PHASE_A_STAGED
  for (uint32_t item = lane; item < QM * nblk; item += WAVE) {
    const uint32_t blk = item / QM, j = item - blk * QM;
    sh.symb[8u * blk + j] = rm_gather32<WRAP>(rm, sh.lin, zc2, j * esym + s0 + 32u * blk);
  }
  wave_sync();
  const uint8_t* rows = reinterpret_cast<const uint8_t*>(sh.symb);
  for (uint32_t item = lane; item < 4u * nblk; item += WAVE) {
    const uint32_t blk = item >> 2, m = item & 3u;
    const uint8_t* b   = rows + 32u * blk + (3u - m);
    uint32_t       r8[8];
#pragma unroll
    for (int j = 0; j != 8; ++j) {
      r8[j] = (j < QM) ? b[4 * j] : 0u;
    }
    uint32_t hi = (r8[0] << 24) | (r8[1] << 16) | (r8[2] << 8) | r8[3];
    uint32_t lo = (r8[4] << 24) | (r8[5] << 16) | (r8[6] << 8) | r8[7];
    transpose8x8(hi, lo);
    sh.symb[8u * blk + 2u * m]      = hi;
    sh.symb[8u * blk + 2u * m + 1u] = lo;
  }
#else
  for (uint32_t blk = lane; blk < nblk; blk += WAVE) {
    uint32_t row[8];
#pragma unroll
    for (int j = 0; j != 8; ++j) {
      row[j] = (j < QM) ? rm_gather32<WRAP>(rm, sh.lin, zc2, (uint32_t)j * esym + s0 + 32u * blk) : 0u;
    }
#pragma unroll
    for (int m = 0; m != 4; ++m) {
      const int sft = 24 - 8 * m;
      uint32_t  hi  = (((row[0] >> sft) & 0xFFu) << 24) | (((row[1] >> sft) & 0xFFu) << 16) |
                    (((row[2] >> sft) & 0xFFu) << 8) | ((row[3] >> sft) & 0xFFu);
      uint32_t lo = (((row[4] >> sft) & 0xFFu) << 24) | (((row[5] >> sft) & 0xFFu) << 16) |
                    (((row[6] >> sft) & 0xFFu) << 8) | ((row[7] >> sft) & 0xFFu);
      transpose8x8(hi, lo);
      sh.symb[8u * blk + 2u * m]      = hi;
      sh.symb[8u * blk + 2u * m + 1u] = lo;
    }
  }
#endif
  if (lane < 8) {
    sh.symb[8u * nblk + lane] = 0;
  }
#pragma unroll
  for (uint32_t k = 0; k != LUT_TRIPS; ++k) {
    if (lane + WAVE * k < (1u << QM)) {
      reinterpret_cast<float2*>(sh.u)[lane + WAVE * k] = lut[k];
    }
  }
  wave_sync();
}

__device__ __forceinline__ void pin_scalar(cf2& w)
{
  asm volatile("" : "+s"(w));
}

struct ChunkMap {
  uint32_t re0;
  uint32_t word0;
  bool     aligned;
  const uint32_t* gwords;
};

template <int QM, int L>
__device__ __forceinline__ uint32_t global_bits(const ChunkGeom& g, const ChunkMap& cm, uint32_t re_count, uint32_t r)
{
  uint32_t bits = 0;
  if (r < re_count) {
    if (QM * L == 32 && cm.aligned) {
      bits = (cm.gwords + cm.word0)[r];
    } else {
      bits = ext32(cm.gwords, g.bit0 + r * (uint32_t)(QM * L));
    }
  }
  return bits;
}
template <int QM, int L>
__device__ __forceinline__ uint32_t x2_bits(const uint32_t* x2, const ChunkGeom& g, const ChunkMap& cm, uint32_t r)
{
  if (QM * L == 32 && cm.aligned) {
    return x2[r];
  }
  return ext32(x2, (g.bit0 & 31u) + r * (uint32_t)(QM * L));
}

template <int QM, int L, bool WORDS>
__device__ __forceinline__ void re_bits(const CbShared& sh, const ChunkGeom& g, const ChunkMap& cm,
                                        uint32_t re_count, uint32_t r, uint32_t& bytes, uint32_t& gbits)
{
  if constexpr (L == 4) {
    bytes = sh.symb[r];
  } else {
    bytes = ext32(sh.symb, 8u * r * L);
  }
  gbits = global_bits<QM, L>(g, cm, re_count, r);
  if constexpr (!WORDS) {
    gbits ^= x2_bits<QM, L>(sh.lin, g, cm, r);
  }
}

template <int QM, int L, int P, bool WORDS>
__device__ __forceinline__ void phase_b_grid(const PdschLaunch& p, PduRef pd, const PduDev* __restrict__ pd_global,
                                             const CbWork& wk, const CbShared& sh, const ChunkGeom& g, const ChunkMap& cm,
                                             uint32_t first_gbits, uint32_t lane, uint32_t* __restrict__ d_grid)
{
  const size_t   grid_base   = (size_t)pd.grid_index * p.grid_nof_ports * NRPHY_NSYMB * p.grid_nof_subc;
  const uint32_t plane_words = NRPHY_NSYMB * p.grid_nof_subc;
  const __amdgpu_buffer_rsrc_t grid_rsrc = __builtin_amdgcn_make_buffer_rsrc(
      d_grid + grid_base, 0, (int)(NRPHY_STAGE(p) == 11 ? 0u : p.grid_nof_ports * plane_words * 4u), 0x00020000);
  cf2 wu[P > 0 ? P : 1][L];
  if constexpr (P > 0) {
    const float NRPHY_CONSTANT* wuni = to_constant(p.weights + pd.weights_offset);
#pragma unroll
    for (int port = 0; port != P; ++port) {
#pragma unroll
      for (int l = 0; l != L; ++l) {
        wu[port][l] = cf2{wuni[2 * (port * L + l)], wuni[2 * (port * L + l) + 1]};
      }
    }
#pragma unroll
    for (int port = 0; port != P; ++port) {
#pragma unroll
      for (int l = 0; l != L; ++l) {
        pin_scalar(wu[port][l]);
      }
    }
  }
  uint32_t l_cur = 0;
#pragma unroll 1
  while (l_cur + 1u < NRPHY_NSYMB && cm.re0 >= pd.sym_re_start[l_cur + 1u]) {
    ++l_cur;
  }
  uint32_t cur_start = pd.sym_re_start[l_cur], cur_end = pd.sym_re_start[l_cur + 1u];
  uint32_t cur_arg = pd.sym_arg[l_cur], cur_row = l_cur * p.grid_nof_subc;
  bool     cur_table = pd.sym_kind[l_cur] == SYM_TABLE;
  uint32_t gbits_next = first_gbits;

  for (uint32_t r0 = 0; r0 < wk.re_count; r0 += WAVE) {
    const uint32_t r        = r0 + lane;
    const uint32_t gcur     = gbits_next;
    gbits_next              = global_bits<QM, L>(g, cm, wk.re_count, r + WAVE);
    const uint32_t re_first = cm.re0 + r0;
    const uint32_t re_last  = re_first + ((wk.re_count - r0 < WAVE ? wk.re_count - r0 : WAVE) - 1u);
    if (re_first >= cur_end && l_cur + 1u < NRPHY_NSYMB) {
#pragma unroll 1
      do {
        ++l_cur;
        cur_start = cur_end;
        cur_end   = pd.sym_re_start[l_cur + 1u];
      } while (re_first >= cur_end && l_cur + 1u < NRPHY_NSYMB);
      cur_arg   = pd.sym_arg[l_cur];
      cur_row   = l_cur * p.grid_nof_subc;
      cur_table = pd.sym_kind[l_cur] == SYM_TABLE;
    }
    if (r >= wk.re_count) {
      continue;
    }
    __builtin_assume(r < (uint32_t)RE_CHUNK + WAVE);
    uint32_t gbits = gcur;
    if constexpr (!WORDS) {
      gbits ^= x2_bits<QM, L>(sh.lin, g, cm, r);
    }
    uint32_t bytes;
    if constexpr (L == 4) {
      bytes = sh.symb[r];
    } else {
      bytes = ext32(sh.symb, 8u * r * L);
    }
    const uint32_t re_pdu = re_first + lane;
    uint32_t       subc, word_offset;
    if (re_last < cur_end) {
      subc = cur_arg + (re_pdu - cur_start);
      if (cur_table) {
        subc = (uint32_t)p.re_table[subc];
      }
      word_offset = cur_row + subc;
    } else {
      uint32_t l_sym = l_cur, start = cur_start, end = cur_end;
#pragma unroll 1
      while (re_pdu >= end && l_sym + 1u < NRPHY_NSYMB) {
        ++l_sym;
        start = end;
        end   = pd_global->sym_re_start[l_sym + 1u];
      }
      subc = pd_global->sym_arg[l_sym] + (re_pdu - start);
      if (pd_global->sym_kind[l_sym] == SYM_TABLE) {
        subc = (uint32_t)p.re_table[subc];
      }
      word_offset = l_sym * p.grid_nof_subc + subc;
    }
    cf2 x[L];
#pragma unroll
    for (int l = 0; l != L; ++l) {
      const uint32_t raw   = ((bytes >> (24 - 8 * l)) & 0xFFu) >> (8 - QM);
      const uint32_t idx   = raw ^ ((gbits >> (32 - (l + 1) * QM)) & ((1u << QM) - 1u));
      const float2   point = reinterpret_cast<const float2*>(sh.u)[lds_probe_index(idx, 0)];
      x[l]                 = cf2{point.x, point.y};
    }
    if constexpr (P > 0) {
#pragma unroll
      for (int port = 0; port != P; ++port) {
        cf2 acc = cmul_ref_packed_uniform(x[0], wu[port][0]);
#pragma unroll
        for (int l = 1; l != L; ++l) {
          acc += cmul_ref_packed_uniform(x[l], wu[port][l]);
        }
        __builtin_amdgcn_raw_buffer_store_b32(pack_cbf16(acc.x, acc.y), grid_rsrc, (int)(word_offset * 4u),
                                              (int)(port * plane_words * 4u), NRPHY_GRID_STORE_AUX);
      }
    } else {
      const uint32_t nof_ports = pd.nof_ports;
      uint32_t       prg       = subc / pd.prg_size_subc;
      prg                      = prg >= pd.nof_prg ? pd.nof_prg - 1 : prg;
      const float* w = p.weights + pd.weights_offset + 2u * prg * nof_ports * L;
#pragma unroll 1
      for (uint32_t port = 0; port != nof_ports; ++port) {
        cf2 acc = cmul_ref_packed(x[0], cf2{w[2 * port * L], w[2 * port * L + 1]});
#pragma unroll
        for (int l = 1; l != L; ++l) {
          acc += cmul_ref_packed(x[l], cf2{w[2 * (port * L + l)], w[2 * (port * L + l) + 1]});
        }
        __builtin_amdgcn_raw_buffer_store_b32(pack_cbf16(acc.x, acc.y), grid_rsrc, (int)(word_offset * 4u),
                                              (int)(port * plane_words * 4u), NRPHY_GRID_STORE_AUX);
      }
    }
  }
}

template <int QM, int L, bool WORDS>
__device__ __forceinline__ void phase_b(const PdschLaunch& p, PduRef pd, const PduDev* __restrict__ pd_global,
                                        const CbWork& wk, const CbShared& sh, const ChunkGeom& g, const ChunkMap& cm,
                                        uint32_t first_gbits, uint32_t lane, uint32_t* __restrict__ d_grid,
                                        uint32_t* __restrict__ d_cw_rm, uint32_t* __restrict__ d_cw_scr)
{
  constexpr uint32_t LQ = QM * L;
  if (d_cw_rm != nullptr || d_cw_scr != nullptr) {
    const uint64_t cw_bit0 = pd.cw_bit_offset + g.cw_cb + (uint64_t)wk.re_begin * LQ;
    for (uint32_t r = lane; r < wk.re_count; r += WAVE) {
      uint32_t bytes, gbits;
      re_bits<QM, L, WORDS>(sh, g, cm, wk.re_count, r, bytes, gbits);
      uint32_t v_rm = 0;
#pragma unroll
      for (int l = 0; l != L; ++l) {
        const uint32_t raw = ((bytes >> (24 - 8 * l)) & 0xFFu) >> (8 - QM);
        v_rm |= raw << (32 - (l + 1) * QM);
      }
      if (d_cw_rm) {
        or_bits_global(d_cw_rm, cw_bit0 + (uint64_t)r * LQ, v_rm, LQ);
      }
      if (d_cw_scr) {
        or_bits_global(d_cw_scr, cw_bit0 + (uint64_t)r * LQ, v_rm ^ (gbits & topmask(LQ)), LQ);
      }
    }
  }
  if (d_grid == nullptr) {
    return;
  }
  const uint32_t nof_ports = pd.nof_prg == 1 ? pd.nof_ports : 0u;
  if (nof_ports == 4u) {
    phase_b_grid<QM, L, 4, WORDS>(p, pd, pd_global, wk, sh, g, cm, first_gbits, lane, d_grid);
  } else if (L <= 3 && nof_ports == 3u) {
    phase_b_grid<QM, (L <= 3 ? L : 1), 3, WORDS>(p, pd, pd_global, wk, sh, g, cm, first_gbits, lane, d_grid);
  } else if (L <= 2 && nof_ports == 2u) {
    phase_b_grid<QM, (L <= 2 ? L : 1), 2, WORDS>(p, pd, pd_global, wk, sh, g, cm, first_gbits, lane, d_grid);
  } else if (L == 1 && nof_ports == 1u) {
    phase_b_grid<QM, 1, 1, WORDS>(p, pd, pd_global, wk, sh, g, cm, first_gbits, lane, d_grid);
  } else {
    phase_b_grid<QM, L, 0, WORDS>(p, pd, pd_global, wk, sh, g, cm, first_gbits, lane, d_grid);
  }
}

template <int QM, int L, bool WORDS>
__device__ __forceinline__ void map_chunk(const PdschLaunch& p, PduRef pd, const PduDev* pd_global, const CbWork& wk,
                                          uint32_t item, const CbShared& sh, uint32_t lane, uint32_t* d_grid,
                                          uint32_t* d_cw_rm, uint32_t* d_cw_scr)
{
  const bool is_long = wk.cb >= pd.n_short;
  ChunkGeom  g;
  g.E     = is_long ? pd.e_long : pd.e_short;
  g.cw_cb = is_long ? pd.n_short * pd.e_short + (wk.cb - pd.n_short) * pd.e_long : wk.cb * pd.e_short;
  g.bit0  = g.cw_cb + wk.re_begin * (uint32_t)(QM * L);
  if (NRPHY_STAGE(p) == 3) {
    return;
  }
  ChunkMap cm;
  cm.re0     = g.cw_cb / (uint32_t)(QM * L) + wk.re_begin;
  cm.word0   = g.bit0 >> 5;
  cm.aligned = (g.bit0 & 31u) == 0;
  cm.gwords  = WORDS ? p.scr_seq + pd.scr_word_offset : p.x1_words;
  uint32_t seed_word = 0u;
  if constexpr (!WORDS) {
    const uint32_t seed_slot = pd.seed_first + (item - pd.item_first);
    seed_word                = lane < 31u ? p.scr_seq[(size_t)seed_slot * 32u + lane] : 0u;
  }
  const uint32_t first_gbits = global_bits<QM, L>(g, cm, wk.re_count, lane);
  {
    const RmIndex rm = rm_index_init(pd);
    if (rm.rank0 + g.E > rm.n_valid) {
      phase_a<QM, L, true>(p, pd, wk, sh, g.E, lane);
    } else {
      phase_a<QM, L, false>(p, pd, wk, sh, g.E, lane);
    }
  }
  if (NRPHY_STAGE(p) == 4) {
    return;
  }
  NRPHY_WG_TRACE_MARK(3);
  if constexpr (!WORDS) {
    static_assert((31u + (uint32_t)RE_CHUNK * 32u + 31u) / 32u + 1u <= GOLD_EXPAND_MAX_WORDS, "a work item's scrambling words");
    gold_expand_seed_wave(sh.lin, seed_word, ((g.bit0 & 31u) + wk.re_count * (uint32_t)(QM * L) + 31u) / 32u + 1u, lane);
  }
  phase_b<QM, L, WORDS>(p, pd, pd_global, wk, sh, g, cm, first_gbits, lane, d_grid, d_cw_rm, d_cw_scr);
}

template <int QM, bool WORDS>
__device__ __forceinline__ void map_chunk_layers(const PdschLaunch& p, PduRef pd, const PduDev* pd_global,
                                                 const CbWork& wk, uint32_t item, const CbShared& sh, uint32_t lane,
                                                 uint32_t* d_grid, uint32_t* d_cw_rm, uint32_t* d_cw_scr)
{
  switch (pd.nof_layers) {
    case 1:
      map_chunk<QM, 1, WORDS>(p, pd, pd_global, wk, item, sh, lane, d_grid, d_cw_rm, d_cw_scr);
      break;
    case 2:
      map_chunk<QM, 2, WORDS>(p, pd, pd_global, wk, item, sh, lane, d_grid, d_cw_rm, d_cw_scr);
      break;
    case 3:
      map_chunk<QM, 3, WORDS>(p, pd, pd_global, wk, item, sh, lane, d_grid, d_cw_rm, d_cw_scr);
      break;
    default:
      map_chunk<QM, 4, WORDS>(p, pd, pd_global, wk, item, sh, lane, d_grid, d_cw_rm, d_cw_scr);
      break;
  }
}

template <int L, typename W>
__device__ __forceinline__ void dmrs_port_words(float dr, float di, bool odd, uint32_t port, W w, uint32_t (&word)[(L + 1) / 2])
{
  const float sr = odd ? -dr : dr, si = odd ? -di : di;
#pragma unroll
  for (int g = 0; g != (L + 1) / 2; ++g) {
    float accr, acci;
    cmul_ref(dr, di, w[2 * (port * L + 2 * g)], w[2 * (port * L + 2 * g) + 1], accr, acci);
    if (2 * g + 1 < L) {
      float pr, pi;
      cmul_ref(sr, si, w[2 * (port * L + 2 * g + 1)], w[2 * (port * L + 2 * g + 1) + 1], pr, pi);
      accr = __fadd_rn(accr, pr);
      acci = __fadd_rn(acci, pi);
    }
    word[g] = pack_cbf16(accr, acci);
  }
}

typedef uint32_t u32x2_t __attribute__((ext_vector_type(2)));
typedef uint32_t u32x4_t __attribute__((ext_vector_type(4)));
template <int L>
__device__ __forceinline__ void dmrs_store(uint32_t* out, const uint32_t (&word)[(L + 1) / 2], bool zero_other_group, bool nt = false)
{
  if ((L + 1) / 2 == 2 || zero_other_group) {
    const u32x2_t v = {word[0], (L + 1) / 2 == 2 ? word[(L + 1) / 2 - 1] : 0u};
    if (nt) {
      __builtin_nontemporal_store(v, reinterpret_cast<u32x2_t*>(out));
    } else {
      *reinterpret_cast<u32x2_t*>(out) = v;
    }
  } else if (nt) {
    __builtin_nontemporal_store(word[0], out);
  } else {
    out[0] = word[0];
  }
}

template <int L, typename W>
__device__ __forceinline__ void dmrs_precode(float dr, float di, bool odd, uint32_t P, W w, uint32_t* out,
                                             size_t port_stride, bool zero_other_group)
{
#pragma unroll 1
  for (uint32_t port = 0; port != P; ++port) {
    uint32_t word[(L + 1) / 2];
    dmrs_port_words<L>(dr, di, odd, port, w, word);
    dmrs_store<L>(out + port * port_stride, word, zero_other_group);
  }
}

template <int L>
__device__ __forceinline__ void dmrs_items(const PdschLaunch& p, PduRef pd, const DmrsWork& wk,
                                           uint32_t* __restrict__ d_grid, uint32_t lane, uint32_t* tab)
{
  const uint32_t  P       = pd.nof_ports;
  const uint32_t  ordinal = __popc(pd.dmrs_symbol_mask & ((1u << wk.symbol) - 1u));
  const uint32_t* seq     = p.scr + pd.dmrs_seq_offset + ordinal * pd.dmrs_seq_words;
  const float     a       = pd.dmrs_amplitude;
  const uint32_t  nof_items = (wk.prb_end - wk.prb_begin) * 6u;
  const size_t    port_stride = (size_t)NRPHY_NSYMB * p.grid_nof_subc;
  uint32_t*       row = d_grid + (size_t)pd.grid_index * p.grid_nof_ports * port_stride + (size_t)wk.symbol * p.grid_nof_subc;
  const bool      wideband = pd.nof_prg == 1;
  const bool      zero_other = pd.dmrs_zero_other_group != 0 && p.zero_fill != 0;
  if (wideband) {
    if (lane < 8u) {
      const float dr = (lane & 4u) ? -a : a, di = (lane & 2u) ? -a : a;
#pragma unroll 1
      for (uint32_t port = 0; port != P; ++port) {
        uint32_t word[(L + 1) / 2];
        dmrs_port_words<L>(dr, di, (lane & 1u) != 0, port, to_constant(p.weights + pd.dmrs_weights_offset), word);
        tab[(lane * NRPHY_MAX_PORTS + port) * 2u]      = word[0];
        tab[(lane * NRPHY_MAX_PORTS + port) * 2u + 1u] = word[(L + 1) / 2 - 1];
      }
    }
    wave_sync();
  }
  for (uint32_t item = lane; item < nof_items; item += WAVE) {
    const uint32_t prb = wk.prb_begin + item / 6u;
    const uint32_t kp  = item % 6u;
    if (!((pd.prb_mask[prb >> 5] >> (prb & 31u)) & 1u)) {
      continue;
    }
    const uint32_t bit  = 12u * (prb - pd.dmrs_ref_rb) + 2u * kp;
    const uint32_t word = seq[bit >> 5] << (bit & 31u);
    uint32_t*      out  = row + 12u * prb + 2u * kp;
    if (wideband) {
      const uint32_t variant = ((word >> 29) & 6u) | (kp & 1u);
#pragma unroll 1
      for (uint32_t port = 0; port != P; ++port) {
        uint32_t words[(L + 1) / 2];
        words[0] = tab[(variant * NRPHY_MAX_PORTS + port) * 2u];
        if ((L + 1) / 2 == 2) {
          words[(L + 1) / 2 - 1] = tab[(variant * NRPHY_MAX_PORTS + port) * 2u + 1u];
        }
        dmrs_store<L>(out + port * port_stride, words, zero_other, p.extras_nt != 0);
      }
      continue;
    }
    const float dr = (word & 0x80000000u) ? -a : a;
    const float di = (word & 0x40000000u) ? -a : a;
    uint32_t    prg = (12u * prb) / pd.prg_size_subc;
    prg             = prg >= pd.nof_prg ? pd.nof_prg - 1 : prg;
    dmrs_precode<L>(dr, di, (kp & 1u) != 0, P, p.weights + pd.dmrs_weights_offset + 2u * prg * P * L, out, port_stride,
                    zero_other);
  }
}

__device__ __forceinline__ void dmrs_wave(const PdschLaunch& p, uint32_t item_index, uint32_t* __restrict__ d_grid,
                                          uint32_t lane, uint32_t* tab)
{
  const auto*    wkc = to_constant(&p.dmrs_work[item_index]);
  const DmrsWork wk  = {wkc->pdu, wkc->symbol, wkc->prb_begin, wkc->prb_end};
  PduRef         pd  = *to_constant(&p.pdus[wk.pdu]);
  switch (pd.nof_layers) {
    case 1:
      dmrs_items<1>(p, pd, wk, d_grid, lane, tab);
      break;
    case 2:
      dmrs_items<2>(p, pd, wk, d_grid, lane, tab);
      break;
    case 3:
      dmrs_items<3>(p, pd, wk, d_grid, lane, tab);
      break;
    default:
      dmrs_items<4>(p, pd, wk, d_grid, lane, tab);
      break;
  }
}

__device__ __forceinline__ void zero_wave(const PdschLaunch& p, uint32_t item_index, uint32_t* __restrict__ d_grid, uint32_t lane)
{
  const auto*    wkc  = to_constant(&p.zero_work[item_index]);
  const uint32_t seg_begin = wkc->seg_begin, seg_count = wkc->seg_count, seg_long = wkc->seg_long;
  uint32_t*      base = d_grid + ((size_t)wkc->grid * p.grid_nof_ports + wkc->port) * NRPHY_NSYMB * p.grid_nof_subc;
  static_assert(sizeof(ZeroSeg) == 8, "one run descriptor per lane as two dwords");
  for (uint32_t first = 0; first < seg_long; first += WAVE) {
    const uint32_t n = seg_long - first < WAVE ? seg_long - first : WAVE;
    uint2          d = make_uint2(0u, 0u);
    if (lane < n) {
      d = *reinterpret_cast<const uint2*>(&p.zero_segs[seg_begin + first + lane]);
    }
    for (uint32_t i = 0; i != n; ++i) {
      const uint32_t lo_word = (uint32_t)__builtin_amdgcn_readlane((int)d.x, (int)i);
      const uint32_t count   = (uint32_t)__builtin_amdgcn_readlane((int)d.y, (int)i) & 0xFFFFu;
      uint32_t*      row     = base + (size_t)(lo_word & 0xFFFFu) * p.grid_nof_subc + (lo_word >> 16);
      const uint32_t off      = (uint32_t)((reinterpret_cast<uintptr_t>(row) >> 2) & 3u);
      uint32_t*      aligned  = row - off;
      const uint32_t n_chunks = (off + count + 3u) >> 2;
      for (uint32_t c = lane; c < n_chunks; c += WAVE) {
        const uint32_t lo = 4u * c;
        if (lo >= off && lo + 4u <= off + count) {
          if (p.extras_nt != 0) {
          __builtin_nontemporal_store(u32x4_t{0u, 0u, 0u, 0u}, reinterpret_cast<u32x4_t*>(aligned + lo));
        } else {
          *reinterpret_cast<uint4*>(aligned + lo) = make_uint4(0u, 0u, 0u, 0u);
        }
        } else {
#pragma unroll
          for (uint32_t w = 0; w != 4; ++w) {
            if (lo + w >= off && lo + w < off + count) {
              aligned[lo + w] = 0u;
            }
          }
        }
      }
    }
  }
  for (uint32_t i = seg_long + lane; i < seg_count; i += WAVE) {
    const ZeroSeg  sg  = p.zero_segs[seg_begin + i];
    uint32_t*      row = base + (size_t)sg.symbol * p.grid_nof_subc + sg.k0;
    for (uint32_t k = 0; k != sg.count; ++k) {
      row[k] = 0u;
    }
  }
}


#ifndef NRPHY_CB_WAVES
#define NRPHY_CB_WAVES 4
#endif
constexpr uint32_t CB_WAVES = NRPHY_CB_WAVES;

struct CbWave {
  uint32_t  lane;
  uint32_t  wave;
  uint32_t* lds;
};
__device__ __forceinline__ CbWave cb_wave(const PdschLaunch& p, uint32_t* dyn_lds)
{
  CbWave w;
  w.lane = threadIdx.x % WAVE;
  w.wave = (uint32_t)__builtin_amdgcn_readfirstlane((int)(threadIdx.x / WAVE));
  w.lds  = dyn_lds + w.wave * (p.lds_lin_words + p.lds_u_words);
  return w;
}
__host__ __device__ __forceinline__ uint32_t cb_blocks(uint32_t n_units)
{
  return (n_units + CB_WAVES - 1u) / CB_WAVES;
}

__device__ __forceinline__ bool extra_wave(const PdschLaunch& p, const CbWave& w, uint32_t* __restrict__ d_grid)
{
  const uint32_t nb = cb_blocks(p.n_work);
  if (blockIdx.x < nb) {
    return false;
  }
  const uint32_t extra = (blockIdx.x - nb) * CB_WAVES + w.wave;
  if (extra < p.n_dmrs_in_launch) {
    dmrs_wave(p, extra, d_grid, w.lane, w.lds);
  } else if (extra - p.n_dmrs_in_launch < p.n_zero_work) {
    zero_wave(p, extra - p.n_dmrs_in_launch, d_grid, w.lane);
  }
  return true;
}

__device__ __forceinline__ uint32_t xcd_work_item(uint32_t n_work, const CbWave& w)
{
  const uint32_t nb  = cb_blocks(n_work);
  const uint32_t xcd = blockIdx.x & 7u, turn = blockIdx.x >> 3;
  const uint32_t q = nb >> 3, r = nb & 7u;
  const uint32_t item = (xcd * q + (xcd < r ? xcd : r) + turn) * CB_WAVES + w.wave;
  return item < n_work ? item : n_work;
}

__device__ __forceinline__ bool codeblock_front(const PdschLaunch& p, PduRef pd, const CbWork& wk, CbShared& sh,
                                                const uint8_t* __restrict__ d_tb, uint32_t lane)
{
  const uint32_t zc = pd.zc, kb = pd.kb;
  if (NRPHY_STAGE(p) == 5 || NRPHY_STAGE(p) == 6) {
    return false;
  }
  const uint32_t total_words = (((kb + pd.nof_rows) * zc + 31u) >> 5) + 2u;
  GraphRows rows;
  rows.fetch(&p.graphs[pd.graph], pd.nof_rows, lane);
  build_codeblock(pd, wk.cb, reinterpret_cast<const uint32_t*>(d_tb + pd.tb_offset), p.tb_crc_part, p.gold, &sh,
                  total_words, lane, NRPHY_STAGE(p));
  if (NRPHY_STAGE(p) == 1 || NRPHY_STAGE(p) == 7) {
    return false;
  }
  NRPHY_WG_TRACE_MARK(1);
  rows.store(pd.nof_rows, sh.graph, lane);
  ldpc_encode_wave(&p.graphs[pd.graph], sh.graph, kb, zc, pd.nof_rows, sh.lin, sh.u, sh.ldpc, lane);
  NRPHY_WG_TRACE_MARK(2);
  return NRPHY_STAGE(p) != 2;
}

template <int QM, int L, bool WORDS>
__device__ __forceinline__ void codeblock_wave_t(const PdschLaunch& p, const uint8_t* __restrict__ d_tb,
                                                 uint32_t* __restrict__ d_grid, uint32_t* __restrict__ d_cw_rm,
                                                 uint32_t* __restrict__ d_cw_scr, uint32_t* dyn_lds)
{
  const CbWave   w    = cb_wave(p, dyn_lds);
  const uint32_t lane = w.lane;
  CbShared       sh;
  sh.lin   = w.lds;
  sh.u     = w.lds + p.lds_lin_words;
  sh.symb  = sh.u + CB_U_QAM_WORDS;
  sh.graph = sh.u + CB_U_GRAPH_OFFSET;
  sh.ldpc  = reinterpret_cast<LdpcScratch*>(sh.u + LDPC_DBL_WORDS);
  if (NRPHY_STAGE(p) == 10 || extra_wave(p, w, d_grid)) {
    return;
  }
  const uint32_t item = xcd_work_item(p.n_work, w);
  if (item == p.n_work) {
    return;
  }
  NRPHY_WG_TRACE_MARK(0);
  NRPHY_WG_TRACE_WHERE(3);
  const auto*  wkc = to_constant(&p.work[item]);
  const CbWork wk  = {wkc->pdu, wkc->cb, wkc->re_begin, wkc->re_count};
  PduRef       pd  = *to_constant(&p.pdus[wk.pdu]);
  if (!codeblock_front(p, pd, wk, sh, d_tb, lane)) {
    return;
  }
  map_chunk<QM, L, WORDS>(p, pd, &p.pdus[wk.pdu], wk, p.work_base + item, sh, lane, d_grid, d_cw_rm, d_cw_scr);
  NRPHY_WG_TRACE_MARK(6);
}

template <int QM, int L>
__global__ __launch_bounds__(WAVE * CB_WAVES) void codeblock_kernel_t(PdschLaunch p, const uint8_t* __restrict__ d_tb,
                                                              uint32_t* __restrict__ d_grid, uint32_t* __restrict__ d_cw_rm,
                                                              uint32_t* __restrict__ d_cw_scr)
{
  extern __shared__ __attribute__((aligned(16))) uint32_t dyn_lds[];
  codeblock_wave_t<QM, L, false>(p, d_tb, d_grid, d_cw_rm, d_cw_scr, dyn_lds);
}
template <int QM, int L>
__global__ __launch_bounds__(WAVE * CB_WAVES) void codeblock_words_kernel_t(PdschLaunch p, const uint8_t* __restrict__ d_tb,
                                                                    uint32_t* __restrict__ d_grid, uint32_t* __restrict__ d_cw_rm,
                                                                    uint32_t* __restrict__ d_cw_scr)
{
  extern __shared__ __attribute__((aligned(16))) uint32_t dyn_lds[];
  codeblock_wave_t<QM, L, true>(p, d_tb, d_grid, d_cw_rm, d_cw_scr, dyn_lds);
}

template <bool WORDS>
__device__ __forceinline__ void codeblock_wave_mixed(const PdschLaunch& p, const uint8_t* __restrict__ d_tb,
                                                     uint32_t* __restrict__ d_grid, uint32_t* __restrict__ d_cw_rm,
                                                     uint32_t* __restrict__ d_cw_scr, uint32_t* dyn_lds)
{
  const CbWave   w    = cb_wave(p, dyn_lds);
  const uint32_t lane = w.lane;
  CbShared       sh;
  sh.lin   = w.lds;
  sh.u     = w.lds + p.lds_lin_words;
  sh.symb  = sh.u + CB_U_QAM_WORDS;
  sh.graph = sh.u + CB_U_GRAPH_OFFSET;
  sh.ldpc  = reinterpret_cast<LdpcScratch*>(sh.u + LDPC_DBL_WORDS);
  if (NRPHY_STAGE(p) == 10 || extra_wave(p, w, d_grid)) {
    return;
  }
  const uint32_t item = xcd_work_item(p.n_work, w);
  if (item == p.n_work) {
    return;
  }
  const auto*  wkc = to_constant(&p.work[item]);
  const CbWork wk  = {wkc->pdu, wkc->cb, wkc->re_begin, wkc->re_count};
  PduRef       pd  = *to_constant(&p.pdus[wk.pdu]);
  if (!codeblock_front(p, pd, wk, sh, d_tb, lane)) {
    return;
  }
  switch (pd.qm) {
    case 2:
      map_chunk_layers<2, WORDS>(p, pd, &p.pdus[wk.pdu], wk, p.work_base + item, sh, lane, d_grid, d_cw_rm, d_cw_scr);
      break;
    case 4:
      map_chunk_layers<4, WORDS>(p, pd, &p.pdus[wk.pdu], wk, p.work_base + item, sh, lane, d_grid, d_cw_rm, d_cw_scr);
      break;
    case 6:
      map_chunk_layers<6, WORDS>(p, pd, &p.pdus[wk.pdu], wk, p.work_base + item, sh, lane, d_grid, d_cw_rm, d_cw_scr);
      break;
    default:
      map_chunk_layers<8, WORDS>(p, pd, &p.pdus[wk.pdu], wk, p.work_base + item, sh, lane, d_grid, d_cw_rm, d_cw_scr);
      break;
  }
}

__global__ __launch_bounds__(WAVE * CB_WAVES) void codeblock_kernel(PdschLaunch p, const uint8_t* __restrict__ d_tb,
                                                         uint32_t* __restrict__ d_grid, uint32_t* __restrict__ d_cw_rm,
                                                         uint32_t* __restrict__ d_cw_scr)
{
  extern __shared__ __attribute__((aligned(16))) uint32_t dyn_lds[];
  codeblock_wave_mixed<false>(p, d_tb, d_grid, d_cw_rm, d_cw_scr, dyn_lds);
}
__global__ __launch_bounds__(WAVE * CB_WAVES) void codeblock_words_kernel(PdschLaunch p, const uint8_t* __restrict__ d_tb,
                                                               uint32_t* __restrict__ d_grid, uint32_t* __restrict__ d_cw_rm,
                                                               uint32_t* __restrict__ d_cw_scr)
{
  extern __shared__ __attribute__((aligned(16))) uint32_t dyn_lds[];
  codeblock_wave_mixed<true>(p, d_tb, d_grid, d_cw_rm, d_cw_scr, dyn_lds);
}

typedef void (*CodeblockKernel)(PdschLaunch, const uint8_t*, uint32_t*, uint32_t*, uint32_t*);

static CodeblockKernel bucket_kernel(uint32_t bucket, bool words)
{
  static const CodeblockKernel seeds_table[CB_BUCKETS] = {
      codeblock_kernel_t<2, 1>, codeblock_kernel_t<2, 2>, codeblock_kernel_t<2, 3>, codeblock_kernel_t<2, 4>,
      codeblock_kernel_t<4, 1>, codeblock_kernel_t<4, 2>, codeblock_kernel_t<4, 3>, codeblock_kernel_t<4, 4>,
      codeblock_kernel_t<6, 1>, codeblock_kernel_t<6, 2>, codeblock_kernel_t<6, 3>, codeblock_kernel_t<6, 4>,
      codeblock_kernel_t<8, 1>, codeblock_kernel_t<8, 2>, codeblock_kernel_t<8, 3>, codeblock_kernel_t<8, 4>};
  static const CodeblockKernel words_table[CB_BUCKETS] = {
      codeblock_words_kernel_t<2, 1>, codeblock_words_kernel_t<2, 2>, codeblock_words_kernel_t<2, 3>, codeblock_words_kernel_t<2, 4>,
      codeblock_words_kernel_t<4, 1>, codeblock_words_kernel_t<4, 2>, codeblock_words_kernel_t<4, 3>, codeblock_words_kernel_t<4, 4>,
      codeblock_words_kernel_t<6, 1>, codeblock_words_kernel_t<6, 2>, codeblock_words_kernel_t<6, 3>, codeblock_words_kernel_t<6, 4>,
      codeblock_words_kernel_t<8, 1>, codeblock_words_kernel_t<8, 2>, codeblock_words_kernel_t<8, 3>, codeblock_words_kernel_t<8, 4>};
  return words ? words_table[bucket] : seeds_table[bucket];
}

bool codeblocks_take_bucket_launches(const PdschLaunch& p, const uint32_t* bucket_begin, int dispatch, uint32_t* nof_buckets)
{
  uint32_t n = 0;
  for (uint32_t b = 0; b != CB_BUCKETS; ++b) {
    n += bucket_begin[b + 1] != bucket_begin[b] ? 1u : 0u;
  }
  *nof_buckets = n;
  return !(dispatch == 1 || (dispatch == 0 && n > 1 && p.n_work < CB_MIXED_MAX_WORK));
}

hipError_t launch_codeblocks(const PdschLaunch& p, const uint32_t* bucket_begin, int dispatch, const uint8_t* d_tb,
                             uint32_t* d_grid, uint32_t* d_cw_rm, uint32_t* d_cw_scr, const hipStream_t* streams, uint32_t n_streams)
{
  if (p.n_work == 0) {
    return hipSuccess;
  }
  const size_t   lds_bytes = 4u * (size_t)(p.lds_lin_words + p.lds_u_words) * CB_WAVES;
  const uint32_t extras    = d_grid ? p.n_dmrs_in_launch + p.n_zero_work : 0u;
  uint32_t       nof_buckets = 0;
  if (!codeblocks_take_bucket_launches(p, bucket_begin, dispatch, &nof_buckets)) {
    hipLaunchKernelGGL(p.scr_as_words != 0 ? codeblock_words_kernel : codeblock_kernel, dim3(cb_blocks(p.n_work) + cb_blocks(extras)),
                       dim3(WAVE * CB_WAVES), lds_bytes, streams[0], p, d_tb, d_grid, d_cw_rm, d_cw_scr);
    return hipGetLastError();
  }
  uint32_t order[CB_BUCKETS], n_order = 0;
  for (uint32_t b = 0; b != CB_BUCKETS; ++b) {
    if (bucket_begin[b + 1] != bucket_begin[b]) {
      uint32_t k = n_order++;
      for (; k != 0 && bucket_begin[order[k - 1] + 1] - bucket_begin[order[k - 1]] < bucket_begin[b + 1] - bucket_begin[b]; --k) {
        order[k] = order[k - 1];
      }
      order[k] = b;
    }
  }
  for (uint32_t i = 0; i != n_order; ++i) {
    const uint32_t b = order[i], n = bucket_begin[b + 1] - bucket_begin[b];
    PdschLaunch    q = p;
    q.work           = p.work + bucket_begin[b];
    q.work_base      = bucket_begin[b];
    q.n_work         = n;
    if (i != 0) {
      q.n_dmrs_in_launch = 0;
      q.n_zero_work      = 0;
    }
    const uint32_t blocks = cb_blocks(n) + (i == 0 ? cb_blocks(extras) : 0u);
    hipLaunchKernelGGL(bucket_kernel(b, p.scr_as_words != 0), dim3(blocks), dim3(WAVE * CB_WAVES), lds_bytes, streams[n_streams > 1 ? i % n_streams : 0], q,
                       d_tb, d_grid, d_cw_rm, d_cw_scr);
    const hipError_t e = hipGetLastError();
    if (e != hipSuccess) {
      return e;
    }
  }
  return hipSuccess;
}

__global__ __launch_bounds__(WAVE) void dmrs_kernel(PdschLaunch p, uint32_t* __restrict__ d_grid)
{
  __shared__ uint32_t tab[8 * NRPHY_MAX_PORTS * 2];
  dmrs_wave(p, blockIdx.x, d_grid, threadIdx.x, tab);
}

hipError_t launch_dmrs(const PdschLaunch& p, uint32_t* d_grid, hipStream_t stream)
{
  if (p.n_dmrs_work == 0) {
    return hipSuccess;
  }
  hipLaunchKernelGGL(dmrs_kernel, dim3(p.n_dmrs_work), dim3(WAVE), 0, stream, p, d_grid);
  return hipGetLastError();
}

__global__ __launch_bounds__(WAVE) void ldpc_encode_kernel(const LiftedGraph* graphs, uint32_t graph, uint32_t kb,
                                                           uint32_t zc, const uint8_t* __restrict__ d_msg,
                                                           uint32_t msg_stride, uint32_t out_bits,
                                                           uint8_t* __restrict__ d_out, uint32_t out_stride)
{
  __shared__ uint32_t    lin[LDPC_LIN_WORDS];
  __shared__ uint32_t    gbuf[LDPC_GRAPH_ROWPTR + MAX_BG_EDGES];
  __shared__ uint32_t    dbl[LDPC_DBL_WORDS];
  __shared__ LdpcScratch scratch;
  const uint32_t         lane = threadIdx.x;
  const uint8_t*         msg  = d_msg + (size_t)blockIdx.x * msg_stride;
  uint8_t*               out  = d_out + (size_t)blockIdx.x * out_stride;

  const uint32_t K   = kb * zc;
  uint32_t       len = out_bits + 2u * zc;
  len                = len < (kb + 4u) * zc ? (kb + 4u) * zc : len;
  const uint32_t nof_rows    = (len + zc - 1u) / zc - kb;
  const uint32_t total_words = (((kb + nof_rows) * zc + 31u) >> 5) + 2u;
  const uint32_t msg_bytes   = (K + 7u) >> 3;
  for (uint32_t j = lane; j < total_words; j += WAVE) {
    uint32_t v = 0;
    for (uint32_t k = 0; k != 4; ++k) {
      uint32_t byte = 4u * j + k;
      v             = (v << 8) | (byte < msg_bytes ? (uint32_t)msg[byte] : 0u);
    }
    uint32_t pos = 32u * j;
    v            = pos >= K ? 0u : (K - pos < 32u ? v & topmask(K - pos) : v);
    lin[j]       = v;
  }
  stage_graph(&graphs[graph], nof_rows, gbuf, lane);
  wave_sync();
  ldpc_encode_wave(&graphs[graph], gbuf, kb, zc, nof_rows, lin, dbl, &scratch, lane);
  const uint32_t out_bytes = (out_bits + 7u) >> 3;
  for (uint32_t j = lane; 4u * j < out_bytes; j += WAVE) {
    uint32_t v   = ext32(lin, 2u * zc + 32u * j);
    uint32_t pos = 32u * j;
    if (out_bits - pos < 32u) {
      v &= topmask(out_bits - pos);
    }
    for (uint32_t k = 0; k != 4 && 4u * j + k < out_bytes; ++k) {
      out[4u * j + k] = (uint8_t)(v >> (24 - 8 * k));
    }
  }
}

hipError_t launch_ldpc_encode(const LiftedGraph* graphs, uint32_t graph, uint32_t kb, uint32_t zc, uint32_t n_cb,
                              const uint8_t* d_msg, uint32_t msg_stride, uint32_t out_bits, uint8_t* d_out,
                              uint32_t out_stride, hipStream_t stream)
{
  if (n_cb == 0) {
    return hipSuccess;
  }
  hipLaunchKernelGGL(ldpc_encode_kernel, dim3(n_cb), dim3(WAVE), 0, stream, graphs, graph, kb, zc, d_msg, msg_stride,
                     out_bits, d_out, out_stride);
  return hipGetLastError();
}

}
```

Baseline: 1.297 million.

## Hoist LDPC core constants and scrambling words out of encoder and RE loops

The LDPC core shift parameters are now read up front as two scalar words before encoding, instead of through the graph pointer inside the parity stage. The divide-by-wpb magic number is computed once on the host and passed in, and it replaces an integer division in the extension-row loop. Scrambling words for a chunk are prefetched into registers (ScrSpan) and written or XORed into LDS before the RE loop, so the mapping loop no longer issues global loads or waits on them. A disassembly checker script is added to verify that no stray loads or waits remain in those loops.

Result: no change. 1.305 million, median of 6 (+0.7%).

```diff
diff --git a/profiles/check_wave_waits.py b/profiles/check_wave_waits.py
--- /dev/null
+++ b/profiles/check_wave_waits.py
@@ -0,0 +1,236 @@
+#!/usr/bin/env python3
+import json
+import os
+import re
+import subprocess
+import sys
+
+sys.path.insert(0, os.path.dirname(os.path.abspath(__file__)))
+import disasm_lib
+
+KERNELS = ("codeblock_kernel_t", "codeblock_words_kernel_t")
+VM_LOAD = re.compile(r"^(global_load|buffer_load|flat_load|scratch_load)")
+VM_WAIT = re.compile(r"^s_waitcnt\b.*vmcnt")
+BRANCH = re.compile(r"^(s_cbranch_\w+|s_branch)\b")
+MUL24 = re.compile(r"^v_(mul|mad)_u32_u24")
+
+
+def kernels(lib):
+    out = {}
+    for co in disasm_lib.code_objects(lib):
+        text = subprocess.run([os.path.join(disasm_lib.LLVM, "llvm-objdump"), "-d", co], capture_output=True, text=True).stdout
+        for m in re.finditer(r"^[0-9a-f]+ <(\S+)>:\n(.*?)(?=^[0-9a-f]+ <|\Z)", text, re.S | re.M):
+            name = disasm_lib.demangle(m.group(1))
+            if not any(name.split("nrphy::")[-1].startswith(k + "<") for k in KERNELS):
+                continue
+            ins = []
+            for line in m.group(2).split("\n"):
+                mm = re.match(r"^\s+(\S.*?)\s*// ([0-9A-Fa-f]+): [0-9A-Fa-f ]+(?:<\S+\+0x([0-9a-f]+)>)?", line)
+                if mm:
+                    ins.append((int(mm.group(2), 16), mm.group(1), mm.group(3)))
+            base = ins[0][0]
+            out[name.replace("void ", "")] = [(a, t, base + int(off, 16) if off and BRANCH.match(t) else None) for a, t, off in ins]
+    return out
+
+
+class Cfg:
+
+    def __init__(self, ins):
+        self.ins = ins
+        index = {a: i for i, (a, _, _) in enumerate(ins)}
+        leaders = {0}
+        for i, (_, t, target) in enumerate(ins):
+            if BRANCH.match(t):
+                leaders.add(index[target])
+                leaders.add(i + 1)
+            elif t.startswith("s_endpgm"):
+                leaders.add(i + 1)
+        starts = sorted(l for l in leaders if l < len(ins))
+        self.blocks = [(s, e) for s, e in zip(starts, starts[1:] + [len(ins)])]
+        first = {s: b for b, (s, _) in enumerate(self.blocks)}
+        self.block_of = {}
+        for b, (s, e) in enumerate(self.blocks):
+            for i in range(s, e):
+                self.block_of[i] = b
+        self.succ = [[] for _ in self.blocks]
+        for b, (s, e) in enumerate(self.blocks):
+            _, t, target = ins[e - 1]
+            if BRANCH.match(t):
+                self.succ[b].append(first[index[target]])
+                if not t.startswith("s_branch") and e in first:
+                    self.succ[b].append(first[e])
+            elif not t.startswith("s_endpgm") and e in first:
+                self.succ[b].append(first[e])
+        self.pred = [[] for _ in self.blocks]
+        for b, ss in enumerate(self.succ):
+            for s in ss:
+                self.pred[s].append(b)
+
+    def loops(self):
+        n = len(self.blocks)
+        order, seen, stack = [], {0}, [(0, iter(self.succ[0]))]
+        while stack:
+            b, it = stack[-1]
+            for s in it:
+                if s not in seen:
+                    seen.add(s)
+                    stack.append((s, iter(self.succ[s])))
+                    break
+            else:
+                order.append(b)
+                stack.pop()
+        order.reverse()
+        full = (1 << n) - 1
+        dom = {b: full for b in order}
+        dom[0] = 1
+        changed = True
+        while changed:
+            changed = False
+            for b in order[1:]:
+                d = full
+                for q in self.pred[b]:
+                    if q in dom:
+                        d &= dom[q]
+                d |= 1 << b
+                if d != dom[b]:
+                    dom[b], changed = d, True
+        loops = {}
+        for b in order:
+            for header in self.succ[b]:
+                if dom[b] >> header & 1:
+                    body, work = loops.setdefault(header, {header}), [b]
+                    while work:
+                        x = work.pop()
+                        if x not in body and x in dom:
+                            body.add(x)
+                            work.extend(self.pred[x])
+        return loops
+
+    def texts(self, blocks):
+        return [(i, self.ins[i][1]) for b in sorted(blocks) for i in range(*self.blocks[b])]
+
+
+def next_vm_wait(cfg, i, body):
+    b = cfg.block_of[i]
+    for j in range(i + 1, cfg.blocks[b][1]):
+        if VM_WAIT.match(cfg.ins[j][1]):
+            return {j}
+    found, seen, work = set(), {b}, [s for s in cfg.succ[b] if s in body]
+    while work:
+        s = work.pop()
+        if s in seen:
+            continue
+        seen.add(s)
+        hit = next((j for j in range(*cfg.blocks[s]) if VM_WAIT.match(cfg.ins[j][1])), None)
+        if hit is not None:
+            found.add(hit)
+        else:
+            work.extend(x for x in cfg.succ[s] if x in body)
+    return found
+
+
+def analyse(ins):
+    cfg = Cfg(ins)
+    loops = cfg.loops()
+    has_store = {h: body for h, body in loops.items() if any("buffer_store_dword" in t for _, t in cfg.texts(body))}
+    outer = {h: body for h, body in has_store.items() if not any(h2 != h and body < b2 for h2, b2 in has_store.items())}
+    re_loops = []
+    for h, body in sorted(outer.items()):
+        inner = set()
+        for h2, b2 in has_store.items():
+            if h2 != h and b2 < body:
+                inner |= b2
+        allowed_loads, allowed_waits = set(), set()
+        for i, t in cfg.texts(body):
+            if VM_LOAD.match(t) and (t.startswith("global_load_ushort") or cfg.block_of[i] in inner):
+                allowed_loads.add(i)
+                allowed_waits |= next_vm_wait(cfg, i, body)
+        loads = [i for i, t in cfg.texts(body) if VM_LOAD.match(t)]
+        waits = [i for i, t in cfg.texts(body) if VM_WAIT.match(t)]
+        re_loops.append({
+            "header": "0x%x" % (ins[cfg.blocks[h][0]][0] - ins[0][0]),
+            "kind": "weights per PRG" if inner else "wideband weights",
+            "blocks": len(body),
+            "instructions": len(cfg.texts(body)),
+            "stores": sum("buffer_store_dword" in t for _, t in cfg.texts(body)),
+            "vm_loads": len(loads),
+            "vm_waits": len(waits),
+            "table_or_weight_loads": len(allowed_loads),
+            "stray_loads": [ins[i][1] for i in loads if i not in allowed_loads],
+            "stray_waits": [ins[i][1] for i in waits if i not in allowed_waits],
+        })
+    gather = -1
+    for i in range(len(ins) - 5):
+        offs = [re.match(r"global_load_dword \S+ \S+ off(?: offset:(\d+))?$", ins[i + k][1].replace(",", "")) for k in range(6)]
+        if all(offs) and [int(m.group(1) or 0) for m in offs] == [64 * k for k in range(6)]:
+            gather = i + 5
+    in_loop = set().union(*loops.values()) if loops else set()
+    mul = [i for i, (_, t, _) in enumerate(ins) if gather >= 0 and i > gather and MUL24.match(t) and cfg.block_of[i] in in_loop]
+    lds_or = [i for i, (_, t, _) in enumerate(ins) if t.startswith("ds_or_b32")]
+    enc = {"found": bool(mul and lds_or and mul[0] < lds_or[-1])}
+    if enc["found"]:
+        sect = [t for _, t, _ in ins[mul[0]:lds_or[-1] + 1]]
+        enc.update(instructions=len(sect), mul24=sum(bool(MUL24.match(t)) for t in sect), lds_or=sum(t.startswith("ds_or_b32") for t in sect),
+                   global_loads=[t for t in sect if VM_LOAD.match(t)], vm_waits=sum(bool(VM_WAIT.match(t)) for t in sect),
+                   rcp=sum(t.startswith("v_rcp") for t in sect))
+    return {"re_loops": re_loops, "encoder": enc, "instructions": len(ins),
+            "vm_waits_kernel": sum(bool(VM_WAIT.match(t)) for _, t, _ in ins)}
+
+
+def check(lib):
+    res = {r[0].replace("void ", ""): r[1:] for r in disasm_lib.resources(lib)}
+    report, failures = {}, []
+    for name, ins in sorted(kernels(lib).items()):
+        a = analyse(ins)
+        a["resources"] = dict(zip(("sgpr", "vgpr", "sgpr_spill", "vgpr_spill", "scratch", "lds"), res.get(name, ("?",) * 6)))
+        report[name] = a
+        if not a["re_loops"]:
+            failures.append("%s: no RE loop found" % name)
+        for l in a["re_loops"]:
+            if l["stray_loads"] or (l["stray_waits"] and l["kind"] == "wideband weights"):
+                failures.append("%s: RE loop at %s (%s): stray loads %s, stray waits %s" % (name, l["header"], l["kind"], l["stray_loads"], l["stray_waits"]))
+        if not a["encoder"]["found"]:
+            failures.append("%s: LDPC encoder section not found" % name)
+        elif a["encoder"]["global_loads"]:
+            failures.append("%s: global loads in the LDPC encoder: %s" % (name, a["encoder"]["global_loads"]))
+        r = a["resources"]
+        if r["sgpr_spill"] != "0" or r["vgpr_spill"] != "0" or r["scratch"] != "0" or int(r["vgpr"]) > 64:
+            failures.append("%s: registers %s" % (name, r))
+    return report, failures
+
+
+def main():
+    args = sys.argv[1:]
+    lib = os.path.join(disasm_lib.ROOT, "srsran-edgeric-5g_amd", "csrc", "libmi355nrphy.so")
+    if "--lib" in args:
+        lib = args[args.index("--lib") + 1]
+    report, failures = check(lib)
+    if "--json" in args:
+        print(json.dumps({"report": report, "failures": failures}, indent=1))
+    else:
+        for name, a in report.items():
+            r = a["resources"]
+            print("%s: %d instructions, SGPR %s VGPR %s, spills %s/%s, scratch %s, static LDS %s, vmcnt waits in the kernel %d" % (
+                name, a["instructions"], r["sgpr"], r["vgpr"], r["sgpr_spill"], r["vgpr_spill"], r["scratch"], r["lds"], a["vm_waits_kernel"]))
+            for l in a["re_loops"]:
+                print("  RE loop at +%s (%s): %d blocks, %d instructions, %d stores; vector-memory loads %d (table / weights %d), vmcnt waits %d; stray loads %d, stray waits %d" % (
+                    l["header"], l["kind"], l["blocks"], l["instructions"], l["stores"], l["vm_loads"], l["table_or_weight_loads"], l["vm_waits"],
+                    len(l["stray_loads"]), len(l["stray_waits"])))
+                for t in l["stray_loads"] + l["stray_waits"]:
+                    print("      stray: " + t)
+            e = a["encoder"]
+            if e["found"]:
+                print("  LDPC encoder: %d instructions (%d 24-bit multiplies, %d LDS ORs), global loads %d, vmcnt waits %d, v_rcp %d" % (
+                    e["instructions"], e["mul24"], e["lds_or"], len(e["global_loads"]), e["vm_waits"], e["rcp"]))
+                for t in e["global_loads"]:
+                    print("      load: " + t)
+            else:
+                print("  LDPC encoder: section not found")
+        print("%d kernels, %d failures" % (len(report), len(failures)))
+        for f in failures:
+            print("FAIL " + f)
+    return 1 if failures else 0
+
+
+if __name__ == "__main__":
+    sys.exit(main())
diff --git a/srsran-edgeric-5g_amd/csrc/ldpc_device.h b/srsran-edgeric-5g_amd/csrc/ldpc_device.h
--- a/srsran-edgeric-5g_amd/csrc/ldpc_device.h
+++ b/srsran-edgeric-5g_amd/csrc/ldpc_device.h
@@ -1,6 +1,8 @@
 #pragma once
 
 #include "bits_device.h"
+
+#include <cstddef>
 
 namespace nrphy {
 
@@ -61,6 +63,28 @@
   }
 }
 
+struct LdpcCore {
+  uint32_t b, s0, s3, mid;
+  __device__ __forceinline__ void fetch(const LiftedGraph* g)
+  {
+    static_assert(offsetof(LiftedGraph, core_b) % 4 == 0 && offsetof(LiftedGraph, core_s0) == offsetof(LiftedGraph, core_b) + 2 &&
+                      offsetof(LiftedGraph, core_s3) == offsetof(LiftedGraph, core_b) + 4 &&
+                      offsetof(LiftedGraph, core_mid) == offsetof(LiftedGraph, core_b) + 6,
+                  "the four numbers are read as two words");
+    const uint32_t NRPHY_CONSTANT* w = reinterpret_cast<const uint32_t NRPHY_CONSTANT*>(&to_constant(g)->core_b);
+    const uint32_t w0 = w[0], w1 = w[1];
+    b   = w0 & 0xFFFFu;
+    s0  = w0 >> 16;
+    s3  = w1 & 0xFFFFu;
+    mid = w1 >> 16;
+  }
+};
+
+__host__ __device__ __forceinline__ uint32_t ldpc_wpb_magic(uint32_t wpb)
+{
+  return (65536u + wpb - 1u) / wpb;
+}
+
 struct GraphRows {
   static constexpr uint32_t TRIPS = (MAX_BG_EDGES + WAVE - 1) / WAVE;
   uint32_t row_ptr, nedges, edge[TRIPS];
@@ -128,9 +152,9 @@
   return acc;
 }
 
-__device__ __forceinline__ void ldpc_double_blocks(const uint32_t* lin, uint32_t kb, uint32_t wpb, uint32_t* dbl, uint32_t lane)
-{
-  const uint32_t magic = (65536u + wpb - 1u) / wpb;
+__device__ __forceinline__ void ldpc_double_blocks(const uint32_t* lin, uint32_t kb, uint32_t wpb, uint32_t magic, uint32_t* dbl,
+                                                   uint32_t lane)
+{
   for (uint32_t item = lane; item < kb * wpb; item += WAVE) {
     const uint32_t n = __umul24(item, magic) >> 16;
     const uint32_t v = lin[item];
@@ -140,15 +164,14 @@
 }
 
 template <bool ALIGNED>
-__device__ inline void ldpc_encode_wave_impl(const LiftedGraph* g, const uint32_t* gbuf, uint32_t kb, uint32_t zc,
+__device__ inline void ldpc_encode_wave_impl(const LdpcCore& core, uint32_t wpb_magic, const uint32_t* gbuf, uint32_t kb, uint32_t zc,
                                              uint32_t nof_rows, uint32_t* lin, uint32_t* dbl, LdpcScratch* sc, uint32_t lane)
 {
   const uint32_t wpb = (zc + 31u) >> 5;
   if (ALIGNED) {
-    ldpc_double_blocks(lin, kb, wpb, dbl, lane);
+    ldpc_double_blocks(lin, kb, wpb, wpb_magic, dbl, lane);
     wave_sync();
   }
-  const uint32_t wpb_magic = (65536u + wpb - 1u) / wpb;
   for (uint32_t item = lane; item < 4u * wpb; item += WAVE) {
     const uint32_t m = __umul24(item, wpb_magic) >> 16, j = item - __umul24(m, wpb);
     sc->aux[m][j] = ALIGNED ? core_row_word_dbl(gbuf, dbl, m, j) : row_word<ALIGNED>(gbuf, lin, zc, m, j);
@@ -164,15 +187,15 @@
   wave_sync();
   uint32_t p0w = 0;
   if (lane < wpb) {
-    uint32_t b = g->core_b;
+    const uint32_t b = core.b;
     p0w        = rot_word<ALIGNED>(sc->sum, 0, zc, b == 0 ? 0 : zc - b, lane);
     sc->p0[lane] = p0w;
   }
   wave_sync();
   if (lane < wpb) {
-    uint32_t p1 = sc->aux[0][lane] ^ rot_word<ALIGNED>(sc->p0, 0, zc, g->core_s0, lane);
-    uint32_t p3 = sc->aux[3][lane] ^ rot_word<ALIGNED>(sc->p0, 0, zc, g->core_s3, lane);
-    uint32_t p2 = (g->core_mid == 1) ? (sc->aux[2][lane] ^ p3) : (sc->aux[1][lane] ^ p1);
+    uint32_t p1 = sc->aux[0][lane] ^ rot_word<ALIGNED>(sc->p0, 0, zc, core.s0, lane);
+    uint32_t p3 = sc->aux[3][lane] ^ rot_word<ALIGNED>(sc->p0, 0, zc, core.s3, lane);
+    uint32_t p2 = (core.mid == 1) ? (sc->aux[2][lane] ^ p3) : (sc->aux[1][lane] ^ p1);
     put_block_word<ALIGNED>(lin, kb + 0, zc, lane, p0w);
     put_block_word<ALIGNED>(lin, kb + 1, zc, lane, p1);
     put_block_word<ALIGNED>(lin, kb + 2, zc, lane, p2);
@@ -181,21 +204,21 @@
   wave_sync();
   uint32_t ext_items = (nof_rows > 4u ? nof_rows - 4u : 0u) * wpb;
   for (uint32_t item = lane; item < ext_items; item += WAVE) {
-    uint32_t m = item / wpb, j = item - m * wpb;
+    uint32_t m = __umul24(item, wpb_magic) >> 16, j = item - __umul24(m, wpb);
     m += 4u;
     put_block_word<ALIGNED>(lin, kb + m, zc, j, row_word<ALIGNED>(gbuf, lin, zc, m, j));
   }
   wave_sync();
 }
 
-__device__ inline void ldpc_encode_wave(const LiftedGraph* g, const uint32_t* gbuf, uint32_t kb, uint32_t zc,
+__device__ inline void ldpc_encode_wave(const LdpcCore& core, uint32_t wpb_magic, const uint32_t* gbuf, uint32_t kb, uint32_t zc,
                                         uint32_t nof_rows, uint32_t* lin, uint32_t* dbl, LdpcScratch* sc, uint32_t lane)
 {
   if ((zc & 31u) == 0) {
-    ldpc_encode_wave_impl<true>(g, gbuf, kb, zc, nof_rows, lin, dbl, sc, lane);
+    ldpc_encode_wave_impl<true>(core, wpb_magic, gbuf, kb, zc, nof_rows, lin, dbl, sc, lane);
   } else {
-    ldpc_encode_wave_impl<false>(g, gbuf, kb, zc, nof_rows, lin, dbl, sc, lane);
-  }
-}
-
-}
+    ldpc_encode_wave_impl<false>(core, wpb_magic, gbuf, kb, zc, nof_rows, lin, dbl, sc, lane);
+  }
+}
+
+}
diff --git a/srsran-edgeric-5g_amd/csrc/nrphy_host.cpp b/srsran-edgeric-5g_amd/csrc/nrphy_host.cpp
--- a/srsran-edgeric-5g_amd/csrc/nrphy_host.cpp
+++ b/srsran-edgeric-5g_amd/csrc/nrphy_host.cpp
@@ -1008,6 +1008,7 @@
     pd.grid_index     = g;
     pd.graph          = (pdu.ldpc_base_graph - 1) * NOF_LIFTING_SIZES + (uint32_t)lifting_position(d.lifting_size);
     pd.zc             = d.lifting_size;
+    pd.wpb_magic      = (65536U + (d.lifting_size + 31U) / 32U - 1U) / ((d.lifting_size + 31U) / 32U);
     pd.kb             = kb;
     pd.K              = d.segment_length;
     pd.info_bits      = d.cb_info_bits;
diff --git a/srsran-edgeric-5g_amd/csrc/nrphy_internal.h b/srsran-edgeric-5g_amd/csrc/nrphy_internal.h
--- a/srsran-edgeric-5g_amd/csrc/nrphy_internal.h
+++ b/srsran-edgeric-5g_amd/csrc/nrphy_internal.h
@@ -98,6 +98,7 @@
   uint32_t end_prb;
   uint32_t crc_first;
   uint32_t crc_count;
+  uint32_t wpb_magic;
 };
 
 struct CbWork {
diff --git a/srsran-edgeric-5g_amd/csrc/pdsch_kernels.hip b/srsran-edgeric-5g_amd/csrc/pdsch_kernels.hip
--- a/srsran-edgeric-5g_amd/csrc/pdsch_kernels.hip
+++ b/srsran-edgeric-5g_amd/csrc/pdsch_kernels.hip
@@ -219,6 +219,7 @@
 #if NRPHY_CRC_SLICES == 4
   const uint4 crc_tab3 = crc_src[lane + 3 * WAVE];
 #endif
+  const uint32_t tb_crc_share = (last && lane < pd.crc_count) ? tb_crc_part[pd.crc_first + lane] : 0u;
   constexpr uint32_t SEG_UNROLL = 5;
   for (uint32_t base = lane; base < total_words; base += WAVE * SEG_UNROLL) {
     uint32_t hi[SEG_UNROLL], lo[SEG_UNROLL];
@@ -266,7 +267,7 @@
     return;
   }
   if (last) {
-    const uint32_t tb_crc = wave_xor(lane < pd.crc_count ? tb_crc_part[pd.crc_first + lane] : 0u);
+    const uint32_t tb_crc = wave_xor(tb_crc_share);
     if (lane == 0) {
       or_bits_lds_exclusive(sh->lin, used, tb_crc << (32u - pd.tb_crc_bits), pd.tb_crc_bits);
     }
@@ -513,52 +514,70 @@
 
 struct ChunkMap {
   uint32_t re0;
-  uint32_t word0;
   bool     aligned;
-  const uint32_t* gwords;
 };
 
+constexpr uint32_t SCR_SPAN_MAX_WORDS = (31u + (uint32_t)RE_CHUNK * 32u + 31u) / 32u + 1u;
+static_assert(SCR_SPAN_MAX_WORDS <= GOLD_EXPAND_MAX_WORDS, "a work item's scrambling words");
+__device__ __forceinline__ uint32_t scr_span_words(uint32_t bit0, uint32_t re_count, uint32_t lq)
+{
+  return ((bit0 & 31u) + re_count * lq + 31u) / 32u + 1u;
+}
+
+struct ScrSpan {
+  static constexpr uint32_t TRIPS = (SCR_SPAN_MAX_WORDS + WAVE - 1u) / WAVE;
+  uint32_t w[TRIPS];
+  __device__ __forceinline__ void fetch(const uint32_t* __restrict__ src, uint32_t n, uint32_t lane)
+  {
+#pragma unroll
+    for (uint32_t k = 0; k != TRIPS; ++k) {
+      w[k] = lane + WAVE * k < n ? src[lane + WAVE * k] : 0u;
+    }
+  }
+  __device__ __forceinline__ void store(uint32_t* lin, uint32_t n, uint32_t lane) const
+  {
+#pragma unroll
+    for (uint32_t k = 0; k != TRIPS; ++k) {
+      if (lane + WAVE * k < n) {
+        lin[lane + WAVE * k] = w[k];
+      }
+    }
+  }
+  __device__ __forceinline__ void xor_into(uint32_t* lin, uint32_t n, uint32_t lane) const
+  {
+#pragma unroll
+    for (uint32_t k = 0; k != TRIPS; ++k) {
+      if (lane + WAVE * k < n) {
+        lin[lane + WAVE * k] ^= w[k];
+      }
+    }
+  }
+};
+
 template <int QM, int L>
-__device__ __forceinline__ uint32_t global_bits(const ChunkGeom& g, const ChunkMap& cm, uint32_t re_count, uint32_t r)
-{
-  uint32_t bits = 0;
-  if (r < re_count) {
-    if (QM * L == 32 && cm.aligned) {
-      bits = (cm.gwords + cm.word0)[r];
-    } else {
-      bits = ext32(cm.gwords, g.bit0 + r * (uint32_t)(QM * L));
-    }
-  }
-  return bits;
-}
+__device__ __forceinline__ uint32_t scr_bits(const uint32_t* lin, const ChunkGeom& g, const ChunkMap& cm, uint32_t r)
+{
+  if (QM * L == 32 && cm.aligned) {
+    return lin[r];
+  }
+  return ext32(lin, (g.bit0 & 31u) + r * (uint32_t)(QM * L));
+}
+
 template <int QM, int L>
-__device__ __forceinline__ uint32_t x2_bits(const uint32_t* x2, const ChunkGeom& g, const ChunkMap& cm, uint32_t r)
-{
-  if (QM * L == 32 && cm.aligned) {
-    return x2[r];
-  }
-  return ext32(x2, (g.bit0 & 31u) + r * (uint32_t)(QM * L));
-}
-
-template <int QM, int L, bool WORDS>
-__device__ __forceinline__ void re_bits(const CbShared& sh, const ChunkGeom& g, const ChunkMap& cm,
-                                        uint32_t re_count, uint32_t r, uint32_t& bytes, uint32_t& gbits)
+__device__ __forceinline__ void re_bits(const CbShared& sh, const ChunkGeom& g, const ChunkMap& cm, uint32_t r, uint32_t& bytes,
+                                        uint32_t& gbits)
 {
   if constexpr (L == 4) {
     bytes = sh.symb[r];
   } else {
     bytes = ext32(sh.symb, 8u * r * L);
   }
-  gbits = global_bits<QM, L>(g, cm, re_count, r);
-  if constexpr (!WORDS) {
-    gbits ^= x2_bits<QM, L>(sh.lin, g, cm, r);
-  }
-}
-
-template <int QM, int L, int P, bool WORDS>
-__device__ __forceinline__ void phase_b_grid(const PdschLaunch& p, PduRef pd, const PduDev* __restrict__ pd_global,
-                                             const CbWork& wk, const CbShared& sh, const ChunkGeom& g, const ChunkMap& cm,
-                                             uint32_t first_gbits, uint32_t lane, uint32_t* __restrict__ d_grid)
+  gbits = scr_bits<QM, L>(sh.lin, g, cm, r);
+}
+
+template <int QM, int L, int P>
+__device__ __forceinline__ void phase_b_grid(const PdschLaunch& p, PduRef pd, const CbWork& wk, const CbShared& sh,
+                                             const ChunkGeom& g, const ChunkMap& cm, uint32_t lane, uint32_t* __restrict__ d_grid)
 {
   const size_t   grid_base   = (size_t)pd.grid_index * p.grid_nof_ports * NRPHY_NSYMB * p.grid_nof_subc;
   const uint32_t plane_words = NRPHY_NSYMB * p.grid_nof_subc;
@@ -587,25 +606,22 @@
   while (l_cur + 1u < NRPHY_NSYMB && cm.re0 >= pd.sym_re_start[l_cur + 1u]) {
     ++l_cur;
   }
-  uint32_t cur_start = pd.sym_re_start[l_cur], cur_end = pd.sym_re_start[l_cur + 1u];
-  uint32_t cur_arg = pd.sym_arg[l_cur], cur_row = l_cur * p.grid_nof_subc;
+  uint32_t cur_end = pd.sym_re_start[l_cur + 1u];
+  uint32_t cur_shift = pd.sym_arg[l_cur] - pd.sym_re_start[l_cur], cur_row = l_cur * p.grid_nof_subc;
   bool     cur_table = pd.sym_kind[l_cur] == SYM_TABLE;
-  uint32_t gbits_next = first_gbits;
-
   for (uint32_t r0 = 0; r0 < wk.re_count; r0 += WAVE) {
     const uint32_t r        = r0 + lane;
-    const uint32_t gcur     = gbits_next;
-    gbits_next              = global_bits<QM, L>(g, cm, wk.re_count, r + WAVE);
     const uint32_t re_first = cm.re0 + r0;
     const uint32_t re_last  = re_first + ((wk.re_count - r0 < WAVE ? wk.re_count - r0 : WAVE) - 1u);
     if (re_first >= cur_end && l_cur + 1u < NRPHY_NSYMB) {
+      uint32_t start;
 #pragma unroll 1
       do {
         ++l_cur;
-        cur_start = cur_end;
-        cur_end   = pd.sym_re_start[l_cur + 1u];
+        start   = cur_end;
+        cur_end = pd.sym_re_start[l_cur + 1u];
       } while (re_first >= cur_end && l_cur + 1u < NRPHY_NSYMB);
-      cur_arg   = pd.sym_arg[l_cur];
+      cur_shift = pd.sym_arg[l_cur] - start;
       cur_row   = l_cur * p.grid_nof_subc;
       cur_table = pd.sym_kind[l_cur] == SYM_TABLE;
     }
@@ -613,10 +629,7 @@
       continue;
     }
     __builtin_assume(r < (uint32_t)RE_CHUNK + WAVE);
-    uint32_t gbits = gcur;
-    if constexpr (!WORDS) {
-      gbits ^= x2_bits<QM, L>(sh.lin, g, cm, r);
-    }
+    const uint32_t gbits = scr_bits<QM, L>(sh.lin, g, cm, r);
     uint32_t bytes;
     if constexpr (L == 4) {
       bytes = sh.symb[r];
@@ -626,24 +639,33 @@
     const uint32_t re_pdu = re_first + lane;
     uint32_t       subc, word_offset;
     if (re_last < cur_end) {
-      subc = cur_arg + (re_pdu - cur_start);
+      subc = cur_shift + re_pdu;
       if (cur_table) {
         subc = (uint32_t)p.re_table[subc];
       }
       word_offset = cur_row + subc;
     } else {
-      uint32_t l_sym = l_cur, start = cur_start, end = cur_end;
+      uint32_t l_sym = l_cur, end = cur_end;
+      uint32_t row = cur_row, shift = cur_shift;
+      uint32_t table = cur_table ? 1u : 0u;
 #pragma unroll 1
-      while (re_pdu >= end && l_sym + 1u < NRPHY_NSYMB) {
+      while (re_last >= end && l_sym + 1u < NRPHY_NSYMB) {
         ++l_sym;
-        start = end;
-        end   = pd_global->sym_re_start[l_sym + 1u];
-      }
-      subc = pd_global->sym_arg[l_sym] + (re_pdu - start);
-      if (pd_global->sym_kind[l_sym] == SYM_TABLE) {
+        const uint32_t start = end;
+        end                  = pd.sym_re_start[l_sym + 1u];
+        const uint32_t arg   = pd.sym_arg[l_sym];
+        const uint32_t kind  = pd.sym_kind[l_sym];
+        if (re_pdu >= start) {
+          row   = l_sym * p.grid_nof_subc;
+          shift = arg - start;
+          table = kind == SYM_TABLE ? 1u : 0u;
+        }
+      }
+      subc = shift + re_pdu;
+      if (table != 0u) {
         subc = (uint32_t)p.re_table[subc];
       }
-      word_offset = l_sym * p.grid_nof_subc + subc;
+      word_offset = row + subc;
     }
     cf2 x[L];
 #pragma unroll
@@ -683,10 +705,9 @@
   }
 }
 
-template <int QM, int L, bool WORDS>
-__device__ __forceinline__ void phase_b(const PdschLaunch& p, PduRef pd, const PduDev* __restrict__ pd_global,
-                                        const CbWork& wk, const CbShared& sh, const ChunkGeom& g, const ChunkMap& cm,
-                                        uint32_t first_gbits, uint32_t lane, uint32_t* __restrict__ d_grid,
+template <int QM, int L>
+__device__ __forceinline__ void phase_b(const PdschLaunch& p, PduRef pd, const CbWork& wk, const CbShared& sh,
+                                        const ChunkGeom& g, const ChunkMap& cm, uint32_t lane, uint32_t* __restrict__ d_grid,
                                         uint32_t* __restrict__ d_cw_rm, uint32_t* __restrict__ d_cw_scr)
 {
   constexpr uint32_t LQ = QM * L;
@@ -694,7 +715,7 @@
     const uint64_t cw_bit0 = pd.cw_bit_offset + g.cw_cb + (uint64_t)wk.re_begin * LQ;
     for (uint32_t r = lane; r < wk.re_count; r += WAVE) {
       uint32_t bytes, gbits;
-      re_bits<QM, L, WORDS>(sh, g, cm, wk.re_count, r, bytes, gbits);
+      re_bits<QM, L>(sh, g, cm, r, bytes, gbits);
       uint32_t v_rm = 0;
 #pragma unroll
       for (int l = 0; l != L; ++l) {
@@ -714,22 +735,21 @@
   }
   const uint32_t nof_ports = pd.nof_prg == 1 ? pd.nof_ports : 0u;
   if (nof_ports == 4u) {
-    phase_b_grid<QM, L, 4, WORDS>(p, pd, pd_global, wk, sh, g, cm, first_gbits, lane, d_grid);
+    phase_b_grid<QM, L, 4>(p, pd, wk, sh, g, cm, lane, d_grid);
   } else if (L <= 3 && nof_ports == 3u) {
-    phase_b_grid<QM, (L <= 3 ? L : 1), 3, WORDS>(p, pd, pd_global, wk, sh, g, cm, first_gbits, lane, d_grid);
+    phase_b_grid<QM, (L <= 3 ? L : 1), 3>(p, pd, wk, sh, g, cm, lane, d_grid);
   } else if (L <= 2 && nof_ports == 2u) {
-    phase_b_grid<QM, (L <= 2 ? L : 1), 2, WORDS>(p, pd, pd_global, wk, sh, g, cm, first_gbits, lane, d_grid);
+    phase_b_grid<QM, (L <= 2 ? L : 1), 2>(p, pd, wk, sh, g, cm, lane, d_grid);
   } else if (L == 1 && nof_ports == 1u) {
-    phase_b_grid<QM, 1, 1, WORDS>(p, pd, pd_global, wk, sh, g, cm, first_gbits, lane, d_grid);
+    phase_b_grid<QM, 1, 1>(p, pd, wk, sh, g, cm, lane, d_grid);
   } else {
-    phase_b_grid<QM, L, 0, WORDS>(p, pd, pd_global, wk, sh, g, cm, first_gbits, lane, d_grid);
+    phase_b_grid<QM, L, 0>(p, pd, wk, sh, g, cm, lane, d_grid);
   }
 }
 
 template <int QM, int L, bool WORDS>
-__device__ __forceinline__ void map_chunk(const PdschLaunch& p, PduRef pd, const PduDev* pd_global, const CbWork& wk,
-                                          uint32_t item, const CbShared& sh, uint32_t lane, uint32_t* d_grid,
-                                          uint32_t* d_cw_rm, uint32_t* d_cw_scr)
+__device__ __forceinline__ void map_chunk(const PdschLaunch& p, PduRef pd, const CbWork& wk, uint32_t item, const CbShared& sh,
+                                          uint32_t lane, uint32_t* d_grid, uint32_t* d_cw_rm, uint32_t* d_cw_scr)
 {
   const bool is_long = wk.cb >= pd.n_short;
   ChunkGeom  g;
@@ -741,15 +761,16 @@
   }
   ChunkMap cm;
   cm.re0     = g.cw_cb / (uint32_t)(QM * L) + wk.re_begin;
-  cm.word0   = g.bit0 >> 5;
   cm.aligned = (g.bit0 & 31u) == 0;
-  cm.gwords  = WORDS ? p.scr_seq + pd.scr_word_offset : p.x1_words;
-  uint32_t seed_word = 0u;
+  const uint32_t  span  = scr_span_words(g.bit0, wk.re_count, (uint32_t)(QM * L));
+  const uint32_t* words = (WORDS ? p.scr_seq + pd.scr_word_offset : p.x1_words) + (g.bit0 >> 5);
+  uint32_t        seed_word = 0u;
   if constexpr (!WORDS) {
     const uint32_t seed_slot = pd.seed_first + (item - pd.item_first);
     seed_word                = lane < 31u ? p.scr_seq[(size_t)seed_slot * 32u + lane] : 0u;
   }
-  const uint32_t first_gbits = global_bits<QM, L>(g, cm, wk.re_count, lane);
+  ScrSpan scr;
+  scr.fetch(words, span, lane);
   {
     const RmIndex rm = rm_index_init(pd);
     if (rm.rank0 + g.E > rm.n_valid) {
@@ -762,30 +783,34 @@
     return;
   }
   NRPHY_WG_TRACE_MARK(3);
-  if constexpr (!WORDS) {
-    static_assert((31u + (uint32_t)RE_CHUNK * 32u + 31u) / 32u + 1u <= GOLD_EXPAND_MAX_WORDS, "a work item's scrambling words");
-    gold_expand_seed_wave(sh.lin, seed_word, ((g.bit0 & 31u) + wk.re_count * (uint32_t)(QM * L) + 31u) / 32u + 1u, lane);
-  }
-  phase_b<QM, L, WORDS>(p, pd, pd_global, wk, sh, g, cm, first_gbits, lane, d_grid, d_cw_rm, d_cw_scr);
+  if constexpr (WORDS) {
+    scr.store(sh.lin, span, lane);
+  } else {
+    gold_expand_seed_wave(sh.lin, seed_word, span, lane);
+    scr.xor_into(sh.lin, span, lane);
+  }
+  wave_sync();
+  __builtin_amdgcn_s_waitcnt(0x0F70);
+  phase_b<QM, L>(p, pd, wk, sh, g, cm, lane, d_grid, d_cw_rm, d_cw_scr);
 }
 
 template <int QM, bool WORDS>
-__device__ __forceinline__ void map_chunk_layers(const PdschLaunch& p, PduRef pd, const PduDev* pd_global,
-                                                 const CbWork& wk, uint32_t item, const CbShared& sh, uint32_t lane,
-                                                 uint32_t* d_grid, uint32_t* d_cw_rm, uint32_t* d_cw_scr)
+__device__ __forceinline__ void map_chunk_layers(const PdschLaunch& p, PduRef pd, const CbWork& wk, uint32_t item,
+                                                 const CbShared& sh, uint32_t lane, uint32_t* d_grid, uint32_t* d_cw_rm,
+                                                 uint32_t* d_cw_scr)
 {
   switch (pd.nof_layers) {
     case 1:
-      map_chunk<QM, 1, WORDS>(p, pd, pd_global, wk, item, sh, lane, d_grid, d_cw_rm, d_cw_scr);
+      map_chunk<QM, 1, WORDS>(p, pd, wk, item, sh, lane, d_grid, d_cw_rm, d_cw_scr);
       break;
     case 2:
-      map_chunk<QM, 2, WORDS>(p, pd, pd_global, wk, item, sh, lane, d_grid, d_cw_rm, d_cw_scr);
+      map_chunk<QM, 2, WORDS>(p, pd, wk, item, sh, lane, d_grid, d_cw_rm, d_cw_scr);
       break;
     case 3:
-      map_chunk<QM, 3, WORDS>(p, pd, pd_global, wk, item, sh, lane, d_grid, d_cw_rm, d_cw_scr);
+      map_chunk<QM, 3, WORDS>(p, pd, wk, item, sh, lane, d_grid, d_cw_rm, d_cw_scr);
       break;
     default:
-      map_chunk<QM, 4, WORDS>(p, pd, pd_global, wk, item, sh, lane, d_grid, d_cw_rm, d_cw_scr);
+      map_chunk<QM, 4, WORDS>(p, pd, wk, item, sh, lane, d_grid, d_cw_rm, d_cw_scr);
       break;
   }
 }
@@ -1029,8 +1054,10 @@
     return false;
   }
   NRPHY_WG_TRACE_MARK(1);
+  LdpcCore core;
+  core.fetch(&p.graphs[pd.graph]);
   rows.store(pd.nof_rows, sh.graph, lane);
-  ldpc_encode_wave(&p.graphs[pd.graph], sh.graph, kb, zc, pd.nof_rows, sh.lin, sh.u, sh.ldpc, lane);
+  ldpc_encode_wave(core, pd.wpb_magic, sh.graph, kb, zc, pd.nof_rows, sh.lin, sh.u, sh.ldpc, lane);
   NRPHY_WG_TRACE_MARK(2);
   return NRPHY_STAGE(p) != 2;
 }
@@ -1063,7 +1090,7 @@
   if (!codeblock_front(p, pd, wk, sh, d_tb, lane)) {
     return;
   }
-  map_chunk<QM, L, WORDS>(p, pd, &p.pdus[wk.pdu], wk, p.work_base + item, sh, lane, d_grid, d_cw_rm, d_cw_scr);
+  map_chunk<QM, L, WORDS>(p, pd, wk, p.work_base + item, sh, lane, d_grid, d_cw_rm, d_cw_scr);
   NRPHY_WG_TRACE_MARK(6);
 }
 
@@ -1112,16 +1139,16 @@
   }
   switch (pd.qm) {
     case 2:
-      map_chunk_layers<2, WORDS>(p, pd, &p.pdus[wk.pdu], wk, p.work_base + item, sh, lane, d_grid, d_cw_rm, d_cw_scr);
+      map_chunk_layers<2, WORDS>(p, pd, wk, p.work_base + item, sh, lane, d_grid, d_cw_rm, d_cw_scr);
       break;
     case 4:
-      map_chunk_layers<4, WORDS>(p, pd, &p.pdus[wk.pdu], wk, p.work_base + item, sh, lane, d_grid, d_cw_rm, d_cw_scr);
+      map_chunk_layers<4, WORDS>(p, pd, wk, p.work_base + item, sh, lane, d_grid, d_cw_rm, d_cw_scr);
       break;
     case 6:
-      map_chunk_layers<6, WORDS>(p, pd, &p.pdus[wk.pdu], wk, p.work_base + item, sh, lane, d_grid, d_cw_rm, d_cw_scr);
+      map_chunk_layers<6, WORDS>(p, pd, wk, p.work_base + item, sh, lane, d_grid, d_cw_rm, d_cw_scr);
       break;
     default:
-      map_chunk_layers<8, WORDS>(p, pd, &p.pdus[wk.pdu], wk, p.work_base + item, sh, lane, d_grid, d_cw_rm, d_cw_scr);
+      map_chunk_layers<8, WORDS>(p, pd, wk, p.work_base + item, sh, lane, d_grid, d_cw_rm, d_cw_scr);
       break;
   }
 }
@@ -1229,7 +1256,7 @@
 }
 
 __global__ __launch_bounds__(WAVE) void ldpc_encode_kernel(const LiftedGraph* graphs, uint32_t graph, uint32_t kb,
-                                                           uint32_t zc, const uint8_t* __restrict__ d_msg,
+                                                           uint32_t zc, uint32_t wpb_magic, const uint8_t* __restrict__ d_msg,
                                                            uint32_t msg_stride, uint32_t out_bits,
                                                            uint8_t* __restrict__ d_out, uint32_t out_stride)
 {
@@ -1257,9 +1284,11 @@
     v            = pos >= K ? 0u : (K - pos < 32u ? v & topmask(K - pos) : v);
     lin[j]       = v;
   }
+  LdpcCore core;
+  core.fetch(&graphs[graph]);
   stage_graph(&graphs[graph], nof_rows, gbuf, lane);
   wave_sync();
-  ldpc_encode_wave(&graphs[graph], gbuf, kb, zc, nof_rows, lin, dbl, &scratch, lane);
+  ldpc_encode_wave(core, wpb_magic, gbuf, kb, zc, nof_rows, lin, dbl, &scratch, lane);
   const uint32_t out_bytes = (out_bits + 7u) >> 3;
   for (uint32_t j = lane; 4u * j < out_bytes; j += WAVE) {
     uint32_t v   = ext32(lin, 2u * zc + 32u * j);
@@ -1280,7 +1309,7 @@
   if (n_cb == 0) {
     return hipSuccess;
   }
-  hipLaunchKernelGGL(ldpc_encode_kernel, dim3(n_cb), dim3(WAVE), 0, stream, graphs, graph, kb, zc, d_msg, msg_stride,
+  hipLaunchKernelGGL(ldpc_encode_kernel, dim3(n_cb), dim3(WAVE), 0, stream, graphs, graph, kb, zc, ldpc_wpb_magic((zc + 31u) >> 5), d_msg, msg_stride,
                      out_bits, d_out, out_stride);
   return hipGetLastError();
 }
```
